# p1an-lin-jung/WavThruVec_pytorch

Measured on AMD Instinct MI355X. Metric: audio samples/sec (16 kHz) Vec2Wav generator, B=32×256-frame 768-d latents, 1/2/4/8 GPU, higher is better.
Workload: dtype f32; 1 GPU; BASELINE configs[1]: B=32/GPU x T=256 frames, 768-d latents, upsample (5,4,4,2,2) x320, ResBlock2, train-mode CondBN, f32; global_batch=32, frames=256, parallelism=single GPU

## Files before the change

include/vec2wav_hip.h:

```cpp
#ifndef VEC2WAV_HIP_H
#define VEC2WAV_HIP_H

#include <stdint.h>

#ifdef __cplusplus
extern "C" {
#endif

#define V2W_ABI_VERSION 34

#define V2W_E_ARG      (-1)
#define V2W_E_SHAPE    (-2)
#define V2W_E_ALGO     (-3)

#define V2W_ALGO_AUTO   0
#define V2W_ALGO_DIRECT 1
#define V2W_ALGO_MFMA   2
#define V2W_ALGO_BF16   4
#define V2W_ALGO_SPLIT  3

int         v2w_abi_version(void);
const char* v2w_build_arch(void);

typedef struct { uint64_t magic; char* buf; int32_t cap; int32_t len; } v2w_name_sink;
#define V2W_NAME_SINK_MAGIC 0x5632574e414d4531ull
#define V2W_NAME_SINK_STREAM(sink) ((void*)((uintptr_t)(sink) | (uintptr_t)1))

int v2w_wn_fold_conv (const float* v, const float* g, float* wf, float* scratch,
                      int c_out, int c_in, int k, void* stream);
int v2w_wn_fold_convt(const float* v, const float* g, float* wf, float* scratch,
                      int c_in, int c_out, int k, void* stream);

int v2w_wf_transpose_flip(const float* wf, float* out, int k, int c_in, int c_out, void* stream);
int v2w_wf_gather_transpose(const float* wf, float* out, int k, int c_in, int c_out, int t_start, int t_step, int n, void* stream);

int v2w_pack_mfma(const float* wf, float* wp, int k, int c_in, int c_out, int u, void* stream);
int v2w_pack_mfma_dgrad(const float* wf, float* wp, int k, int c_in, int c_out, void* stream);
int v2w_pack_mfma_batch(const float* wf, float* wp, int k, int c_in, int c_out, int u, int n, void* stream);

typedef struct {
    const float* v; const float* g; float* wp; float* scale;
    int32_t c_in, c_out, k, u, transposed;
    int32_t mf, ck;
    int32_t _pad;
    float* wf;
    float* wpd;
} v2w_fold_desc;
int v2w_fold_plan(v2w_fold_desc* descs, int n, int32_t* starts);
int v2w_fold_pack_batch(const v2w_fold_desc* descs_dev, const int32_t* starts_dev, int n,
                        int nblk_scale, int nblk_pack, int lds_bytes, void* stream);

typedef struct {
    const float* in;   const float* in_a;  const float* in_s;
    const float* wf;
    const float* wp;
    const float* bias;
    const float* res;  const float* res_a; const float* res_s;
    const float* add0; const float* add1;
    const float* mask_src; const float* mask_a; const float* mask_s;
    float*       out;
    int32_t B, C_in, C_out, L, k, dil;
    float   slope;
    int32_t accumulate;
    float   out_div;
    int32_t algo;
    float   mask_slope;
    int32_t in_stride, in_phase;
    int32_t pad_left;
    const void*  wps;
    const float* winv;
    int32_t in_ct, out_ct;
    float   out_slope;
    int32_t io_bf16;
    float*  rowsum_part;
    float*  splitk_ws;
    int64_t splitk_ws_bytes;
} v2w_conv1d_args;
int v2w_conv1d_fwd(const v2w_conv1d_args* a, void* stream);
long long v2w_conv1d_splitk_ws_bytes(const v2w_conv1d_args* a, int n);
int v2w_conv1d_fwd_multi(const v2w_conv1d_args* a, int n, void* stream);

int v2w_split_supported(int c_in, int c_out, int u);
int v2w_split_packable(int c_in, int c_out);
int v2w_pack_split(const float* wf, void* wps, float* sc, int k, int c_in, int c_out, void* stream);
int v2w_pack_bf16(const float* wf, void* wps, float* sc, int k, int c_in, int c_out, void* stream);
typedef struct {
    const float* v; const float* g;
    void* wps; float* sc;
    float* rowscale;
    int32_t c_in, c_out, k;
    int32_t mode;
} v2w_split_desc;
int v2w_split_pack_batch(const v2w_split_desc* descs_dev, const int32_t* starts_dev, int n, int nblk_rows, int nblk_pack,
                         int k_max, int all_bf16, void* stream);

typedef struct {
    const float* in; const float* in_a; const float* in_s;
    const float* wp1; const float* bias1; const float* wp2; const float* bias2;
    const float* add0; const float* add1;
    float* out;
    int32_t B, C, L, k, dil1, dil2;
    int32_t res_mode;
    float slope, out_div;
} v2w_pair_args;
int v2w_resblock_pair_fwd(const v2w_pair_args* a, int n, void* stream);

typedef struct {
    const float* in; const float* in_a; const float* in_s;
    const float* wp1[4]; const float* bias1[4]; const float* wp2[4]; const float* bias2[4];
    int32_t k[4], dil1[4], dil2[4];
    float* out;
    int32_t nk, B, C, L;
    float slope, out_div;
    const float* post_w; const float* post_b; float* post_out;
    int32_t post_k;
    float post_slope;
    const float* bwd_mask1[4]; float* bwd_mid[4];
    const float* bwd_mask2; const float* bwd_mask2_a; const float* bwd_mask2_s;
    float bwd_slope;
    float* bwd_rowsum[4];
} v2w_stage_args;
int v2w_resblock2_stage_fwd(const v2w_stage_args* a, void* stream);
int v2w_resblock2_stage_bwd_rows(const v2w_stage_args* a);
int v2w_resblock2_stage_small_fwd(const v2w_stage_args* a, void* stream);

typedef struct {
    const float* in; const float* in_a; const float* in_s;
    const void*  wps1[4]; const float* sc1[4]; const float* bias1[4];
    const void*  wps2[4]; const float* sc2[4]; const float* bias2[4];
    int32_t k[4], dil1[4], dil2[4];
    float* out;
    int32_t nk, B, C, L;
    float slope, out_div;
    int32_t bf16;
    int32_t io_bf16;
    const float* post_w; const float* post_b; float* post_out;
    int32_t post_k;
    float post_slope;
    const void* up_wps; const float* up_bias; void* up_out; float* up_stats_part;
    int32_t up_k, up_u;
    float up_slope;
    int32_t rb1;
    const void* in_b[4]; void* out_b[4];
    const void* add0; const void* add1;
} v2w_stage_split_args;
int v2w_resblock2_stage_split_fwd(const v2w_stage_split_args* a, void* stream);
int v2w_resblock2_stage_split_config(const v2w_stage_split_args* a);
int v2w_resblock2_stage_up_tiles(const v2w_stage_split_args* a);

typedef struct {
    const void* in[3];
    const float* in_a; const float* in_s;
    const void* wps[3]; const float* bias[3];
    void* out[3];
    int32_t k[3], dil[3];
    int32_t nbr, mode, B, C, L;
    float slope, out_div;
    int32_t _pad;
} v2w_branch_convs_args;
int v2w_branch_convs_bf16_fwd(const v2w_branch_convs_args* a, void* stream);

typedef struct {
    const float* in; const float* wf; const float* wp; const float* bias; float* out;
    float* stats_part;
    int32_t B, C_in, C_out, L, k, u;
    float   slope;
    int32_t algo;
    int32_t io_bf16;
    int32_t _pad;
    float*  splitk_ws;
    int64_t splitk_ws_bytes;
} v2w_convt1d_args;
int v2w_convt1d_fwd(const v2w_convt1d_args* a, void* stream);
long long v2w_convt1d_splitk_ws_bytes(const v2w_convt1d_args* a);

int       v2w_pack_bf16_convt(const float* wf, void* wps, int k, int c_in, int c_out, int u, void* stream);
long long v2w_pack_bf16_convt_bytes(int k, int c_in, int c_out, int u);
int       v2w_convt1d_bf16_fwd(const v2w_convt1d_args* a, void* stream);
int       v2w_convt1d_bf16_tiles(const v2w_convt1d_args* a);

int v2w_conv1d_tile_config(const v2w_conv1d_args* a, int32_t* cfg);
int v2w_convt1d_tile_config(const v2w_convt1d_args* a, int32_t* cfg);
int v2w_conv1d_bf16_config(const v2w_conv1d_args* a, int n, int32_t* cfg);
int v2w_convt1d_bf16_config(const v2w_convt1d_args* a, int32_t* cfg);

#define V2W_MAX_STAGES 8
typedef struct {
    const float* spk; const float* noise;
    const float* fc_w[V2W_MAX_STAGES]; const float* fc_b[V2W_MAX_STAGES];
    const float* sn_w[V2W_MAX_STAGES]; const float* sn_b[V2W_MAX_STAGES];
    float* sn_u[V2W_MAX_STAGES]; float* sn_v[V2W_MAX_STAGES];
    float* gb[V2W_MAX_STAGES];
    int32_t C[V2W_MAX_STAGES];
    float* z_ws; float* sigma_ws;
    int32_t n_stages, B, spk_dim, noise_dim, training;
} v2w_cond_args;
int v2w_cond_gamma_beta(const v2w_cond_args* a, void* stream);
int v2w_cond_sigma(const v2w_cond_args* a, void* stream);
typedef struct {
// ... 83 lines not shown
```

wavthruvec_pytorch_amd/_hip.py:

```python
from __future__ import annotations

import ctypes as C
import os
import threading

from . import build as _build

ABI_VERSION = 34
V2W_MAX_STAGES = 8
V2W_BN_SPLITS = 64
ALGO_AUTO, ALGO_DIRECT, ALGO_MFMA, ALGO_SPLIT, ALGO_BF16 = 0, 1, 2, 3, 4

_fp = C.c_void_p


class Conv1dArgs(C.Structure):
    _fields_ = [('in_', _fp), ('in_a', _fp), ('in_s', _fp), ('wf', _fp), ('wp', _fp), ('bias', _fp),
                ('res', _fp), ('res_a', _fp), ('res_s', _fp), ('add0', _fp), ('add1', _fp),
                ('mask_src', _fp), ('mask_a', _fp), ('mask_s', _fp), ('out', _fp),
                ('B', C.c_int32), ('C_in', C.c_int32), ('C_out', C.c_int32), ('L', C.c_int32),
                ('k', C.c_int32), ('dil', C.c_int32), ('slope', C.c_float), ('accumulate', C.c_int32),
                ('out_div', C.c_float), ('algo', C.c_int32), ('mask_slope', C.c_float),
                ('in_stride', C.c_int32), ('in_phase', C.c_int32), ('pad_left', C.c_int32),
                ('wps', _fp), ('winv', _fp), ('in_ct', C.c_int32), ('out_ct', C.c_int32), ('out_slope', C.c_float),
                ('io_bf16', C.c_int32), ('rowsum_part', _fp), ('splitk_ws', _fp), ('splitk_ws_bytes', C.c_int64)]


class ConvT1dArgs(C.Structure):
    _fields_ = [('in_', _fp), ('wf', _fp), ('wp', _fp), ('bias', _fp), ('out', _fp), ('stats_part', _fp),
                ('B', C.c_int32), ('C_in', C.c_int32), ('C_out', C.c_int32), ('L', C.c_int32),
                ('k', C.c_int32), ('u', C.c_int32), ('slope', C.c_float), ('algo', C.c_int32), ('io_bf16', C.c_int32), ('_pad', C.c_int32),
                ('splitk_ws', _fp), ('splitk_ws_bytes', C.c_int64)]


class PairArgs(C.Structure):
    _fields_ = [('in_', _fp), ('in_a', _fp), ('in_s', _fp), ('wp1', _fp), ('bias1', _fp), ('wp2', _fp), ('bias2', _fp),
                ('add0', _fp), ('add1', _fp), ('out', _fp),
                ('B', C.c_int32), ('C', C.c_int32), ('L', C.c_int32), ('k', C.c_int32), ('dil1', C.c_int32), ('dil2', C.c_int32),
                ('res_mode', C.c_int32), ('slope', C.c_float), ('out_div', C.c_float)]


class StageArgs(C.Structure):
    _fields_ = [('in_', _fp), ('in_a', _fp), ('in_s', _fp),
                ('wp1', _fp * 4), ('bias1', _fp * 4), ('wp2', _fp * 4), ('bias2', _fp * 4),
                ('k', C.c_int32 * 4), ('dil1', C.c_int32 * 4), ('dil2', C.c_int32 * 4),
                ('out', _fp), ('nk', C.c_int32), ('B', C.c_int32), ('C', C.c_int32), ('L', C.c_int32),
                ('slope', C.c_float), ('out_div', C.c_float),
                ('post_w', _fp), ('post_b', _fp), ('post_out', _fp), ('post_k', C.c_int32), ('post_slope', C.c_float),
                ('bwd_mask1', _fp * 4), ('bwd_mid', _fp * 4), ('bwd_mask2', _fp), ('bwd_mask2_a', _fp), ('bwd_mask2_s', _fp),
                ('bwd_slope', C.c_float), ('bwd_rowsum', _fp * 4)]


class FoldDesc(C.Structure):
    _fields_ = [('v', _fp), ('g', _fp), ('wp', _fp), ('scale', _fp),
                ('c_in', C.c_int32), ('c_out', C.c_int32), ('k', C.c_int32), ('u', C.c_int32), ('transposed', C.c_int32),
                ('mf', C.c_int32), ('ck', C.c_int32), ('_pad', C.c_int32), ('wf', _fp), ('wpd', _fp)]


_P4 = _fp * 4
_I4 = C.c_int32 * 4


class StageSplitArgs(C.Structure):
    _fields_ = [('in_', _fp), ('in_a', _fp), ('in_s', _fp),
                ('wps1', _P4), ('sc1', _P4), ('bias1', _P4), ('wps2', _P4), ('sc2', _P4), ('bias2', _P4),
                ('k', _I4), ('dil1', _I4), ('dil2', _I4), ('out', _fp),
                ('nk', C.c_int32), ('B', C.c_int32), ('C', C.c_int32), ('L', C.c_int32),
                ('slope', C.c_float), ('out_div', C.c_float), ('bf16', C.c_int32), ('io_bf16', C.c_int32),
                ('post_w', _fp), ('post_b', _fp), ('post_out', _fp), ('post_k', C.c_int32), ('post_slope', C.c_float),
                ('up_wps', _fp), ('up_bias', _fp), ('up_out', _fp), ('up_stats_part', _fp),
                ('up_k', C.c_int32), ('up_u', C.c_int32), ('up_slope', C.c_float), ('rb1', C.c_int32),
                ('in_b', _P4), ('out_b', _P4), ('add0', _fp), ('add1', _fp)]


class BranchConvsArgs(C.Structure):
    _fields_ = [('in_', _fp * 3), ('in_a', _fp), ('in_s', _fp), ('wps', _fp * 3), ('bias', _fp * 3), ('out', _fp * 3),
                ('k', C.c_int32 * 3), ('dil', C.c_int32 * 3),
                ('nbr', C.c_int32), ('mode', C.c_int32), ('B', C.c_int32), ('C', C.c_int32), ('L', C.c_int32),
                ('slope', C.c_float), ('out_div', C.c_float), ('_pad', C.c_int32)]


class SplitDesc(C.Structure):
    _fields_ = [('v', _fp), ('g', _fp), ('wps', _fp), ('sc', _fp), ('rowscale', _fp),
                ('c_in', C.c_int32), ('c_out', C.c_int32), ('k', C.c_int32), ('mode', C.c_int32)]


_PA = _fp * V2W_MAX_STAGES


class CondArgs(C.Structure):
    _fields_ = [('spk', _fp), ('noise', _fp),
                ('fc_w', _PA), ('fc_b', _PA), ('sn_w', _PA), ('sn_b', _PA), ('sn_u', _PA), ('sn_v', _PA),
                ('gb', _PA), ('C', C.c_int32 * V2W_MAX_STAGES), ('z_ws', _fp), ('sigma_ws', _fp),
                ('n_stages', C.c_int32), ('B', C.c_int32), ('spk_dim', C.c_int32), ('noise_dim', C.c_int32),
                ('training', C.c_int32)]


class CondEvalArgs(C.Structure):
    _fields_ = [('c', CondArgs), ('running_mean', _PA), ('running_var', _PA), ('a_out', _PA), ('s_out', _PA),
                ('eps', C.c_float * V2W_MAX_STAGES)]


SIGNATURES = {
    'v2w_abi_version': (C.c_int, []),
    'v2w_build_arch': (C.c_char_p, []),
    'v2w_wn_fold_conv': (C.c_int, [_fp, _fp, _fp, _fp, C.c_int, C.c_int, C.c_int, _fp]),
    'v2w_wn_fold_convt': (C.c_int, [_fp, _fp, _fp, _fp, C.c_int, C.c_int, C.c_int, _fp]),
    'v2w_wf_transpose_flip': (C.c_int, [_fp, _fp, C.c_int, C.c_int, C.c_int, _fp]),
    'v2w_wf_gather_transpose': (C.c_int, [_fp, _fp, C.c_int, C.c_int, C.c_int, C.c_int, C.c_int, C.c_int, _fp]),
    'v2w_pack_mfma': (C.c_int, [_fp, _fp, C.c_int, C.c_int, C.c_int, C.c_int, _fp]),
    'v2w_pack_mfma_batch': (C.c_int, [_fp, _fp, C.c_int, C.c_int, C.c_int, C.c_int, C.c_int, _fp]),
    'v2w_pack_mfma_dgrad': (C.c_int, [_fp, _fp, C.c_int, C.c_int, C.c_int, _fp]),
    'v2w_split_supported': (C.c_int, [C.c_int, C.c_int, C.c_int]),
    'v2w_pack_split': (C.c_int, [_fp, _fp, _fp, C.c_int, C.c_int, C.c_int, _fp]),
    'v2w_mel_phases': (C.c_int, [_fp, _fp, C.c_int, C.c_int, C.c_int, C.c_int, C.c_int, _fp]),
    'v2w_mel_finish': (C.c_int, [_fp, _fp, _fp, C.c_int, C.c_int, C.c_int, C.c_int, C.c_int, C.c_int, _fp]),
    'v2w_mel_finish_bwd': (C.c_int, [_fp, _fp, _fp, _fp, _fp, C.c_int, C.c_int, C.c_int, C.c_int, C.c_int, C.c_int, _fp]),
    'v2w_phase_split': (C.c_int, [_fp, _fp, C.c_int, C.c_int, C.c_int, C.c_int, C.c_int, C.c_int, C.c_int, C.c_int, _fp]),
    'v2w_unfold1': (C.c_int, [_fp, _fp, C.c_int, C.c_int, C.c_int, C.c_int, C.c_int, C.c_int, C.c_int, C.c_int, C.c_int, _fp]),
    'v2w_unfold_taps': (C.c_int, [_fp, _fp] + [C.c_int] * 9 + [_fp]),
    'v2w_wgrad_slice': (C.c_int, [_fp, _fp, _fp, _fp] + [C.c_int] * 9 + [_fp]),
    'v2w_wgrad_group_slabs': (C.c_int, [C.c_int] * 5),
    'v2w_wgrad_groups': (C.c_int, [_fp, _fp, _fp, _fp] + [C.c_int] * 8 + [_fp]),
    'v2w_disc_dz': (C.c_int, [_fp, _fp, _fp, _fp, _fp, C.c_longlong, C.c_int, C.c_int, C.c_float, _fp]),
    'v2w_rowsum_reduce': (C.c_int, [_fp, _fp, C.c_int, C.c_int, _fp]),
    'v2w_disc_dz_merge': (C.c_int, [_fp, _fp, _fp, _fp, _fp] + [C.c_int] * 8 + [C.c_float, _fp]),
    'v2w_phase_merge': (C.c_int, [_fp, _fp] + [C.c_int] * 8 + [_fp]),
    'v2w_fold1': (C.c_int, [_fp, _fp] + [C.c_int] * 9 + [_fp]),
    'v2w_avgpool4_bwd': (C.c_int, [_fp, _fp, C.c_int, C.c_int, _fp]),
    'v2w_cout1_wgrad': (C.c_int, [_fp, _fp, _fp] + [C.c_int] * 6 + [_fp]),
    'v2w_zero_tail': (C.c_int, [_fp, C.c_longlong, C.c_int, C.c_int, _fp]),
    'v2w_avgpool4': (C.c_int, [_fp, _fp, C.c_int, C.c_int, _fp]),
    'v2w_mel_phases_bwd': (C.c_int, [_fp, _fp, C.c_int, C.c_int, C.c_int, C.c_int, C.c_int, _fp]),
    'v2w_split_packable': (C.c_int, [C.c_int, C.c_int]),
    'v2w_resblock2_stage_split_fwd': (C.c_int, [C.POINTER(StageSplitArgs), _fp]),
    'v2w_resblock2_stage_split_config': (C.c_int, [C.POINTER(StageSplitArgs)]),
    'v2w_resblock2_stage_up_tiles': (C.c_int, [C.POINTER(StageSplitArgs)]),
    'v2w_pack_bf16': (C.c_int, [_fp, _fp, _fp, C.c_int, C.c_int, C.c_int, _fp]),
    'v2w_split_pack_batch': (C.c_int, [_fp, _fp, C.c_int, C.c_int, C.c_int, C.c_int, C.c_int, _fp]),
    'v2w_fold_plan': (C.c_int, [C.POINTER(FoldDesc), C.c_int, C.POINTER(C.c_int32)]),
    'v2w_fold_pack_batch': (C.c_int, [_fp, _fp, C.c_int, C.c_int, C.c_int, C.c_int, _fp]),
    'v2w_conv1d_fwd': (C.c_int, [C.POINTER(Conv1dArgs), _fp]),
    'v2w_conv1d_fwd_multi': (C.c_int, [C.POINTER(Conv1dArgs), C.c_int, _fp]),
    'v2w_conv1d_splitk_ws_bytes': (C.c_longlong, [C.POINTER(Conv1dArgs), C.c_int]),
    'v2w_convt1d_splitk_ws_bytes': (C.c_longlong, [C.POINTER(ConvT1dArgs)]),
    'v2w_resblock_pair_fwd': (C.c_int, [C.POINTER(PairArgs), C.c_int, _fp]),
    'v2w_resblock2_stage_bwd_rows': (C.c_int, [C.POINTER(StageArgs)]),
    'v2w_resblock2_stage_fwd': (C.c_int, [C.POINTER(StageArgs), _fp]),
    'v2w_resblock2_stage_small_fwd': (C.c_int, [C.POINTER(StageArgs), _fp]),
    'v2w_branch_convs_bf16_fwd': (C.c_int, [C.POINTER(BranchConvsArgs), _fp]),
    'v2w_convt1d_fwd': (C.c_int, [C.POINTER(ConvT1dArgs), _fp]),
    'v2w_pack_bf16_convt': (C.c_int, [_fp, _fp, C.c_int, C.c_int, C.c_int, C.c_int, _fp]),
    'v2w_pack_bf16_convt_bytes': (C.c_longlong, [C.c_int, C.c_int, C.c_int, C.c_int]),
    'v2w_convt1d_bf16_fwd': (C.c_int, [C.POINTER(ConvT1dArgs), _fp]),
    'v2w_convt1d_bf16_tiles': (C.c_int, [C.POINTER(ConvT1dArgs)]),
    'v2w_conv1d_tile_config': (C.c_int, [C.POINTER(Conv1dArgs), C.POINTER(C.c_int32)]),
    'v2w_convt1d_tile_config': (C.c_int, [C.POINTER(ConvT1dArgs), C.POINTER(C.c_int32)]),
    'v2w_conv1d_bf16_config': (C.c_int, [C.POINTER(Conv1dArgs), C.c_int, C.POINTER(C.c_int32)]),
    'v2w_convt1d_bf16_config': (C.c_int, [C.POINTER(ConvT1dArgs), C.POINTER(C.c_int32)]),
    'v2w_cond_gamma_beta': (C.c_int, [C.POINTER(CondArgs), _fp]),
    'v2w_cond_sigma': (C.c_int, [C.POINTER(CondArgs), _fp]),
    'v2w_cond_affine_eval': (C.c_int, [C.POINTER(CondEvalArgs), _fp]),
    'v2w_bn_stats': (C.c_int, [_fp, _fp, _fp, C.c_int, C.c_int, C.c_int, _fp]),
    'v2w_bn_reduce_partials': (C.c_int, [_fp, C.c_int, C.c_int, C.c_double, _fp, _fp]),
    'v2w_bn_finalize': (C.c_int, [_fp, _fp, _fp, _fp, _fp, _fp, _fp, C.c_int, C.c_int, C.c_int,
                                  C.c_float, C.c_float, _fp]),
    'v2w_bn_reduce_finalize': (C.c_int, [_fp, C.c_int, C.c_double, _fp, _fp, _fp, _fp, _fp, _fp, _fp, C.c_int, C.c_int, C.c_float, C.c_float, _fp]),
    'v2w_bn_reduce_slices': (C.c_int, [_fp, C.c_int, C.c_int, _fp, C.c_int, _fp]),
    'v2w_bn_finalize_slices': (C.c_int, [_fp, C.c_int, C.c_double, _fp, _fp, _fp, _fp, _fp, _fp, C.c_int, C.c_int, C.c_float, C.c_float, _fp]),
    'v2w_affine_apply': (C.c_int, [_fp, _fp, _fp, _fp, C.c_int, C.c_int, C.c_int, _fp]),
    'v2w_wgrad_slabs': (C.c_int, [C.c_int, C.c_int, C.c_int, C.c_int]),
    'v2w_wgrad': (C.c_int, [_fp, _fp, _fp, _fp, _fp, _fp, C.c_int, C.c_int, C.c_int, C.c_int, C.c_int, C.c_int, C.c_int,
                            C.c_float, _fp]),
    'v2w_wgrad_bf16_slabs': (C.c_int, [C.c_int] * 5),
    'v2w_wgrad_bf16': (C.c_int, [_fp] * 6 + [C.c_int] * 6 + [C.c_float, C.c_int, _fp]),
    'v2w_cbn_bwd_sums': (C.c_int, [_fp] * 9 + [C.c_int, C.c_int, C.c_int, C.c_int, C.c_float, _fp]),
    'v2w_cbn_bwd_apply': (C.c_int, [_fp] * 9 + [C.c_int, C.c_int, C.c_int, C.c_int, C.c_float, _fp]),
    'v2w_tail_bwd': (C.c_int, [_fp] * 8 + [C.c_int, C.c_int, C.c_int, C.c_int, C.c_float, _fp]),
    'v2w_wn_bwd': (C.c_int, [_fp] * 5 + [C.c_int, C.c_int, C.c_int, C.c_int, _fp]),
    'v2w_cond_bwd': (C.c_int, [_fp] * 13 + [C.c_int, C.c_int, C.c_int, C.c_int, _fp]),
    'v2w_conv_post_tanh_bf16in': (C.c_int, [_fp, _fp, _fp, _fp, C.c_int, C.c_int, C.c_int, C.c_int, C.c_float, _fp]),
    'v2w_conv_post_tanh': (C.c_int, [_fp, _fp, _fp, _fp, C.c_int, C.c_int, C.c_int, C.c_int, C.c_float, _fp]),
}

LAUNCHERS = frozenset(n for n, (_r, a) in SIGNATURES.items() if a and a[-1] is _fp)

_lib = None
_tls = threading.local()


class HipLibraryError(RuntimeError):

    def __init__(self, msg, code=None):
        super().__init__(msg)
        self.code = code


E_ARG, E_SHAPE, E_ALGO = -1, -2, -3


def lib_path() -> str:
    return os.environ.get('V2W_LIB') or _build.LIB_PATH


def load():
    global _lib
    rec = getattr(_tls, 'recorder', None)
    if rec is not None:
        return rec
    if _lib is not None:
        return _lib
    import torch
    path = lib_path()
    if not os.path.exists(path):
        raise HipLibraryError(
            f'{path} not found: build it with `python -m wavthruvec_pytorch_amd.build` '
            '(or __graft_entry__.build()); there is no CPU/PyTorch fallback for the Vec2Wav hot path')
    lib = C.CDLL(path)
    for name, (res, args) in SIGNATURES.items():
        try:
            fn = getattr(lib, name)
        except AttributeError as e:
            raise HipLibraryError(f'{path} does not export {name}') from e
        fn.restype = res
        fn.argtypes = args
    if lib.v2w_abi_version() != ABI_VERSION:
        raise HipLibraryError(f'ABI version mismatch: library {lib.v2w_abi_version()}, binding {ABI_VERSION}')
    _lib = lib
    return lib


def set_recorder(rec):
    prev = getattr(_tls, 'recorder', None)
    _tls.recorder = rec
    return prev


class NameSink(C.Structure):
    _fields_ = [('magic', C.c_uint64), ('buf', C.c_void_p), ('cap', C.c_int32), ('len', C.c_int32)]


NAME_SINK_MAGIC = 0x5632574e414d4531


def kernel_name_short(full: str) -> str:
    s = full.strip()
    if s.startswith('void '):
        s = s[5:]
    s = s.replace('(anonymous namespace)::', '')
    depth = 0
    for i, ch in enumerate(s):
        if ch == '<':
            depth += 1
        elif ch == '>':
            depth -= 1
        elif ch == '(' and depth == 0:
            return s[:i]
    return s


def kernel_names(fn, *args, short=True):
    buf = C.create_string_buffer(8192)
    sink = NameSink(NAME_SINK_MAGIC, C.addressof(buf), len(buf), 0)
    rc = fn(*args, C.c_void_p(C.addressof(sink) | 1))
    names = [n for n in buf.value.decode().split('\n') if n]
# ... 34 lines not shown
```

wavthruvec_pytorch_amd/build.py:

```python
from __future__ import annotations

import contextlib
import fcntl
import hashlib
import os
import shutil
import subprocess
from concurrent.futures import ThreadPoolExecutor

PKG_DIR = os.path.dirname(os.path.abspath(__file__))
CSRC = os.path.join(PKG_DIR, 'csrc')
OBJ_DIR = os.path.join(CSRC, '_obj')
LIB_PATH = os.path.join(PKG_DIR, 'libvec2wav_hip.so')
SOURCES = ['v2w_api.hip', 'v2w_conv_mfma.hip', 'v2w_conv_split.hip', 'v2w_conv_bf16.hip', 'v2w_conv_bf16_res.hip', 'v2w_convt_bf16_res.hip', 'v2w_stage_split.hip', 'v2w_stage_bf16.hip', 'v2w_stage_bf16_wide.hip', 'v2w_stage_bf16_n16.hip', 'v2w_stage_bf16_n16s.hip', 'v2w_stage_bf16_n32s.hip', 'v2w_resblock_fused.hip', 'v2w_stage_small.hip',
           'v2w_wgrad.hip', 'v2w_wgrad_bf16.hip', 'v2w_backward.hip', 'v2w_direct.hip', 'v2w_conv_post_bf16.hip', 'v2w_cbn.hip', 'v2w_fold.hip', 'v2w_mel.hip', 'v2w_disc.hip']
HEADERS = ['v2w_common.h', 'v2w_tile.h', os.path.join('..', '..', 'include', 'vec2wav_hip.h')]
FLAGS = ['--offload-arch=gfx950', '-O3', '-std=c++17', '-fPIC']


def find_hipcc() -> str:
    for cand in (os.environ.get('HIPCC'), shutil.which('hipcc'), '/opt/rocm/bin/hipcc'):
        if cand and os.path.exists(cand):
            return cand
    raise RuntimeError('hipcc not found (set HIPCC or install ROCm)')


def _obj(src: str) -> str:
    return os.path.join(OBJ_DIR, src + '.o')


def _stale_sources():
    hdr_t = max(os.path.getmtime(os.path.join(CSRC, h)) for h in HEADERS)
    out = []
    for s in SOURCES:
        o = _obj(s)
        if not os.path.exists(o) or os.path.getmtime(o) < max(hdr_t, os.path.getmtime(os.path.join(CSRC, s))):
            out.append(s)
    return out


def needs_build() -> bool:
    if not os.path.exists(LIB_PATH):
        return True
    t = os.path.getmtime(LIB_PATH)
    deps = [os.path.join(CSRC, s) for s in SOURCES + HEADERS]
    return any(os.path.getmtime(d) > t for d in deps)


def sources_hash() -> str:
    hsh = hashlib.sha256()
    for f in sorted(SOURCES) + sorted(HEADERS):
        with open(os.path.join(CSRC, f), 'rb') as fh:
            hsh.update(os.path.basename(f).encode() + b'\0' + fh.read())
    return hsh.hexdigest()[:16]


@contextlib.contextmanager
def _build_lock():
    os.makedirs(OBJ_DIR, exist_ok=True)
    with open(os.path.join(OBJ_DIR, '.lock'), 'w') as lk:
        fcntl.flock(lk, fcntl.LOCK_EX)
        try:
            yield
        finally:
            fcntl.flock(lk, fcntl.LOCK_UN)


def build(force: bool = False, verbose: bool = False, jobs: int | None = None) -> str:
    if not force and not needs_build():
        return LIB_PATH
    hipcc = find_hipcc()
    with _build_lock():
        if not force and not needs_build():
            return LIB_PATH
        todo = list(SOURCES) if force else _stale_sources()

        def run(cmd, what):
            if verbose:
                print(' '.join(cmd), flush=True)
            r = subprocess.run(cmd, capture_output=True, text=True)
            if r.returncode != 0:
                raise RuntimeError(f'{what}:\n' + r.stdout + r.stderr)

        def compile_one(s):
            tmp = _obj(s) + f'.tmp{os.getpid()}'
            try:
                run([hipcc] + FLAGS + ['-c', '-o', tmp, os.path.join(CSRC, s)], f'hipcc failed on {s}')
                os.replace(tmp, _obj(s))
            finally:
                if os.path.exists(tmp):
                    os.remove(tmp)

        jobs = jobs or max(1, min(len(todo) or 1, (os.cpu_count() or 2)))
        with ThreadPoolExecutor(max_workers=jobs) as ex:
            list(ex.map(compile_one, todo))
        tmp = LIB_PATH + f'.tmp{os.getpid()}'
        try:
            run([hipcc, '--offload-arch=gfx950', '-fPIC', '-shared', '-o', tmp] + [_obj(s) for s in SOURCES], 'hipcc link failed')
            os.replace(tmp, LIB_PATH)
        finally:
            if os.path.exists(tmp):
                os.remove(tmp)
    return LIB_PATH


if __name__ == '__main__':
    import sys
    print(build(force='--force' in sys.argv, verbose=True))
```

wavthruvec_pytorch_amd/csrc/v2w_api.hip:

```cpp
#include "v2w_common.h"

int v2w_conv1d_mfma(const v2w_conv1d_args* a, int n, hipStream_t stream, int* cfg_out, long long* ws_query = nullptr);
int v2w_convt1d_mfma(const v2w_convt1d_args* a, hipStream_t stream, int* cfg_out, long long* ws_query = nullptr);
int v2w_conv1d_split(const v2w_conv1d_args* a, int n, hipStream_t stream, bool bf16);
int v2w_conv1d_direct(const v2w_conv1d_args* a, hipStream_t stream);
int v2w_convt1d_direct(const v2w_convt1d_args* a, hipStream_t stream);

extern "C" int v2w_abi_version(void) { return V2W_ABI_VERSION; }
extern "C" const char* v2w_build_arch(void) { return "gfx950"; }

static int check_conv1d(const v2w_conv1d_args* a) {
    if (!a || !a->in || !a->out) return V2W_E_ARG;
    if ((a->algo == V2W_ALGO_SPLIT || a->algo == V2W_ALGO_BF16) ? (!a->wps || !a->winv) : (!a->wf && !a->wp)) return V2W_E_ARG;
    if (a->B <= 0 || a->C_in <= 0 || a->C_out <= 0 || a->L <= 0 || a->k <= 0 || a->dil <= 0) return V2W_E_ARG;
    if ((a->k & 1) == 0 && a->pad_left < 0) return V2W_E_SHAPE;
    if (a->pad_left > a->dil * (a->k - 1) || a->in_stride < 0 || a->in_phase < 0 || (a->in_stride > 0 && a->in_phase >= a->in_stride))
        return V2W_E_ARG;
    if ((a->in_a == nullptr) != (a->in_s == nullptr)) return V2W_E_ARG;
    if ((a->res_a == nullptr) != (a->res_s == nullptr)) return V2W_E_ARG;
    if (a->res_a && !a->res) return V2W_E_ARG;
    if (a->add1 && !a->add0) return V2W_E_ARG;
    if (a->add0 && a->accumulate) return V2W_E_ARG;
    if ((a->mask_a == nullptr) != (a->mask_s == nullptr)) return V2W_E_ARG;
    if (a->mask_a && !a->mask_src) return V2W_E_ARG;
    if (a->in_ct < 0 || a->out_ct < 0 || (a->in_ct > 0 && a->in_ct < a->C_in) || (a->out_ct > 0 && a->out_ct < a->C_out)) return V2W_E_ARG;
    if (((a->in_ct > 0 && a->in_ct != a->C_in) && a->in_a) || ((a->out_ct > 0 && a->out_ct != a->C_out) && (a->res_a || a->mask_a)))
        return V2W_E_ARG;
    if (a->out_slope < 0.f) return V2W_E_ARG;
    if (a->rowsum_part && (a->algo != V2W_ALGO_MFMA || !a->mask_src)) return V2W_E_ARG;
    if (a->io_bf16 != 0 && (a->algo != V2W_ALGO_BF16 || a->io_bf16 < 0 || a->io_bf16 > 3)) return V2W_E_ARG;
    const bool ext_ct = (a->in_ct > 0 && a->in_ct != a->C_in) || (a->out_ct > 0 && a->out_ct != a->C_out);
    const bool ext_slope = a->out_slope != 0.f && a->out_slope != 1.f;
    if ((ext_ct || ext_slope) && a->algo == V2W_ALGO_BF16) return V2W_E_SHAPE;
    return 0;
}

extern "C" int v2w_conv1d_fwd(const v2w_conv1d_args* a, void* stream) {
    if (const int rc = check_conv1d(a)) return rc;
    hipStream_t st = (hipStream_t)stream;
    switch (a->algo) {
        case V2W_ALGO_DIRECT: return a->wf ? v2w_conv1d_direct(a, st) : V2W_E_ARG;
        case V2W_ALGO_MFMA: return v2w_conv1d_mfma(a, 1, st, nullptr);
        case V2W_ALGO_SPLIT: return v2w_conv1d_split(a, 1, st, false);
        case V2W_ALGO_BF16: return v2w_conv1d_split(a, 1, st, true);
        case V2W_ALGO_AUTO: {
            const int rc = v2w_conv1d_mfma(a, 1, st, nullptr);
            return rc == V2W_E_SHAPE ? (a->wf ? v2w_conv1d_direct(a, st) : V2W_E_ARG) : rc;
        }
        default: return V2W_E_ALGO;
    }
}

extern "C" int v2w_convt1d_fwd(const v2w_convt1d_args* a, void* stream) {
    if (!a || !a->in || (!a->wf && !a->wp) || !a->out || a->io_bf16 != 0) return V2W_E_ARG;
    if (a->B <= 0 || a->C_in <= 0 || a->C_out <= 0 || a->L <= 0 || a->k <= 0 || a->u <= 0) return V2W_E_ARG;
    if (a->k < a->u || ((a->k - a->u) & 1)) return V2W_E_SHAPE;
    hipStream_t st = (hipStream_t)stream;
    switch (a->algo) {
        case V2W_ALGO_DIRECT: return (a->wf && !a->stats_part) ? v2w_convt1d_direct(a, st) : V2W_E_ARG;
        case V2W_ALGO_MFMA: return v2w_convt1d_mfma(a, st, nullptr);
        case V2W_ALGO_AUTO: {
            const int rc = v2w_convt1d_mfma(a, st, nullptr);
            return rc == V2W_E_SHAPE ? ((a->wf && !a->stats_part) ? v2w_convt1d_direct(a, st) : V2W_E_ARG) : rc;
        }
        default: return V2W_E_ALGO;
    }
}

extern "C" int v2w_conv1d_tile_config(const v2w_conv1d_args* a, int32_t* cfg) {
    if (!a || !cfg) return V2W_E_ARG;
    return v2w_conv1d_mfma(a, 1, nullptr, cfg);
}
extern "C" int v2w_convt1d_tile_config(const v2w_convt1d_args* a, int32_t* cfg) {
    if (!a || !cfg) return V2W_E_ARG;
    return v2w_convt1d_mfma(a, nullptr, cfg);
}

extern "C" long long v2w_conv1d_splitk_ws_bytes(const v2w_conv1d_args* a, int n) {
    if (!a || n < 1 || n > 4 || (a->algo != V2W_ALGO_AUTO && a->algo != V2W_ALGO_MFMA)) return 0;
    long long bytes = 0;
    return v2w_conv1d_mfma(a, n, nullptr, nullptr, &bytes) == 0 ? bytes : 0;
}
extern "C" long long v2w_convt1d_splitk_ws_bytes(const v2w_convt1d_args* a) {
    if (!a || a->u <= 0 || a->k < a->u || (a->algo != V2W_ALGO_AUTO && a->algo != V2W_ALGO_MFMA)) return 0;
    long long bytes = 0;
    return v2w_convt1d_mfma(a, nullptr, nullptr, &bytes) == 0 ? bytes : 0;
}

extern "C" int v2w_conv1d_fwd_multi(const v2w_conv1d_args* a, int n, void* stream) {
    if (!a || n < 1 || n > 4) return V2W_E_ARG;
    for (int i = 0; i < n; ++i) {
        if (const int rc = check_conv1d(a + i)) return rc;
        if (a[i].algo == V2W_ALGO_DIRECT) return V2W_E_SHAPE;
        if (a[i].algo != a[0].algo && (a[i].algo >= V2W_ALGO_SPLIT || a[0].algo >= V2W_ALGO_SPLIT)) return V2W_E_ARG;
    }
    if (a[0].algo == V2W_ALGO_SPLIT || a[0].algo == V2W_ALGO_BF16)
        return v2w_conv1d_split(a, n, (hipStream_t)stream, a[0].algo == V2W_ALGO_BF16);
    return v2w_conv1d_mfma(a, n, (hipStream_t)stream, nullptr);
}
```

wavthruvec_pytorch_amd/csrc/v2w_conv_mfma.hip:

```cpp
#include <type_traits>
#include "v2w_tile.h"

#ifdef V2W_TIMELINE
V2W_TL_SETTER(v2w_timeline_set_tile)
#endif

namespace {

template <int MF, int CK> struct TileGeom {
    static constexpr int RS = CK == 32 ? 36 : (MF == 32 ? 20 : 24);
    static constexpr int PAIR_DC = MF == 32 ? 2 : 4;
    __host__ __device__ static constexpr int slot(int c) {
        return MF == 32 ? ((c & ~7) + 4 * (c & 1) + ((c & 7) >> 1)) : (4 * (c & 3) + (c >> 2));
    }
    __host__ __device__ static constexpr int pair_c0(int P) {
        return MF == 32 ? (8 * (P >> 2) + 4 * (P & 1) + ((P >> 1) & 1)) : (8 * (P & 1) + (P >> 1));
    }
};

template <int MF, int U, int MI, int NI, int WM, int WN, int CK, int NPF, int RING, int EPI, bool VEC>
__global__ void __launch_bounds__(64 * WM * WN, (U == 1 && MI * NI >= 4) ? 3 : 1)
conv_tile_kernel(const MultiArgs m) {
    typedef Frag<MF> F;
    typedef typename F::acc_t acc_t;
    constexpr int NTHREADS = 64 * WM * WN;
    constexpr int MT = MF * MI * WM;
    constexpr int NT = MF * NI * WN;
    constexpr int KSTEP = F::KSTEP;
    constexpr int CKG = 4 * KSTEP;
    constexpr int GPC = CK / CKG;
    constexpr int RS = TileGeom<MF, CK>::RS;
    static_assert(CK % CKG == 0, "chunk must hold whole A fragments");
    static_assert(RING == 2 || (RING == 4 && GPC == 4), "the 4-deep ring walks exactly one tap per revolution");

    extern __shared__ __attribute__((aligned(16))) float smem[];

    int pq = 0;
#pragma unroll
    for (int i = 1; i < V2W_MAX_MULTI; ++i) pq += (int)blockIdx.x >= m.start[i] ? 1 : 0;
    const TileArgs& p = m.p[pq];
    const int mtiles = p.Cout / MT;
    int id = blockIdx.x - m.start[pq];
    int slice = 0;
    if (p.ksplit > 1) {
        const int per = ((p.ntiles + 7) >> 3) * 8 * mtiles;
        slice = id / per;
        id -= slice * per;
    }
    const int grp = id / (8 * mtiles), rem = id % (8 * mtiles);
    const int mt = rem >> 3;
    const int tile = grp * 8 + (rem & 7);
    if (tile >= p.ntiles) return;
    const int b = tile / p.ntl;
    const int n0 = (tile % p.ntl) * NT;
    const int m0 = mt * MT;

    const int tid = threadIdx.x;
    const int lane = tid & 63;
    const int wave = __builtin_amdgcn_readfirstlane(tid >> 6);
    const int lr = lane & (MF - 1);
    const int hk = lane / MF;
    const int wm0 = (wave / WN) * (MF * MI);
    const int wn0 = (wave % WN) * (MF * NI);
    const int L = p.L, K = p.K;
    const float slope = p.slope;
    const int nch = p.Cin / CK;
    const int nchs = p.ksplit > 1 ? nch / p.ksplit : nch;
    const int ch0 = slice * nchs, ch1 = ch0 + nchs;
    float* const outp = p.out + (size_t)slice * p.B * p.CoutT * L * U;
    const int pos0 = n0 - p.hla;
    const int bufsz = p.xrows * RS;
    float* const etab = smem + p.atab_off;
    float* const atab = etab + 5 * MT;

    V2W_STAMP(0);
    acc_t acc[U][MI][NI];
#pragma unroll
    for (int r = 0; r < U; ++r)
#pragma unroll
        for (int i = 0; i < MI; ++i)
#pragma unroll
            for (int j = 0; j < NI; ++j)
#pragma unroll
                for (int e = 0; e < F::NREG; ++e) acc[r][i][j][e] = 0.f;

    const int nq = p.xrows >> 2;
    const int nq8 = (nq + 7) >> 3;
    const unsigned magic = (unsigned)(((1ull << 32) + nq8 - 1) / nq8);
    f32x4 pf[NPF][2];
    const f32x4 zero4 = {0.f, 0.f, 0.f, 0.f};
    auto item = [&](int s, int& c0, int& row, bool& in_img, bool& in_seq) {
        int t = tid;
        asm volatile("" : "+v"(t));
        const int idx = t + s * NTHREADS;
        const int g = idx >> 4;
        const int pg = (int)__umulhi((unsigned)g, magic);
        const int quad = (g - pg * nq8) * 8 + (idx & 7);
        const int P = 2 * pg + ((idx >> 3) & 1);
        row = quad * 4;
        in_img = quad < nq && P < CK / 2;
        c0 = TileGeom<MF, CK>::pair_c0(in_img ? P : 0);
        const int pos = pos0 + row;
        in_seq = in_img && pos >= 0 && pos < L;
    };
    auto prefetch = [&](int ci0) {
        const float* src = p.in + (size_t)(b * p.CinT + ci0) * L + pos0;
#pragma unroll
        for (int s = 0; s < NPF; ++s) {
            int c0, row; bool in_img, in_seq;
            item(s, c0, row, in_img, in_seq);
            pf[s][0] = zero4; pf[s][1] = zero4;
            if (in_seq) {
                pf[s][0] = *reinterpret_cast<const f32x4*>(src + (size_t)c0 * L + row);
                pf[s][1] = *reinterpret_cast<const f32x4*>(src + (size_t)(c0 + TileGeom<MF, CK>::PAIR_DC) * L + row);
            }
        }
    };
    auto commit = [&](int ci0, float* Xs) {
#pragma unroll
        for (int s = 0; s < NPF; ++s) {
            int c0, row; bool in_img, in_seq;
            item(s, c0, row, in_img, in_seq);
            if (!in_img) continue;
            float a0 = 1.f, s0 = 0.f, a1 = 1.f, s1 = 0.f;
            if (p.in_a) {
                a0 = atab[ci0 + c0]; s0 = atab[p.Cin + ci0 + c0];
                a1 = atab[ci0 + c0 + TileGeom<MF, CK>::PAIR_DC]; s1 = atab[p.Cin + ci0 + c0 + TileGeom<MF, CK>::PAIR_DC];
            }
            float* dst = Xs + row * RS + TileGeom<MF, CK>::slot(c0);
#pragma unroll
            for (int e = 0; e < 4; ++e) {
                f32x2 v = {0.f, 0.f};
                if (in_seq) { v[0] = v2w_lrelu(fmaf(a0, pf[s][0][e], s0), slope); v[1] = v2w_lrelu(fmaf(a1, pf[s][1][e], s1), slope); }
                *reinterpret_cast<f32x2*>(dst + e * RS) = v;
            }
        }
    };
    auto stage_scalar = [&](int ci0, float* Xs) {
        for (int c = wave; c < CK; c += WM * WN) {
            const int ch = b * p.CinT + ci0 + c;
            const float* src = p.in + (size_t)ch * L * p.in_stride + p.in_phase;
            const float av = p.in_a ? p.in_a[ch] : 1.f;
            const float sv = p.in_s ? p.in_s[ch] : 0.f;
            float* dst = Xs + TileGeom<MF, CK>::slot(c);
            for (int j = lane; j < p.xrows; j += 64) {
                const int l = pos0 + j;
                float v = 0.f;
                if (l >= 0 && l < L) v = v2w_lrelu(fmaf(av, src[(size_t)l * p.in_stride], sv), slope);
                dst[j * RS] = v;
            }
        }
    };

    const int nfrag = nch * K * GPC;
// ... 475 lines not shown
            floats += n * s2;
        }
        if (m.p[0].ws_query) {
            *m.p[0].ws_query = ok ? (long long)(floats * sizeof(float)) : 0;
            return 0;
        }
        if (ok && m.p[0].splitk_ws && (long long)(floats * sizeof(float)) <= m.p[0].splitk_ws_bytes) {
            float* ws = m.p[0].splitk_ws;
            {
                S = s2;
                red_vec = vec;
                size_t off = 0;
                long long f4 = 0;
                grid = 0;
                for (int i = 0; i < nprob; ++i) {
                    TileArgs& p = m.p[i];
                    const size_t n = (size_t)p.B * p.Cout * p.L * U;
                    red.e[i] = SplitEpi{ws + off, p.out, p.bias, p.res, p.res_a, p.res_s, p.add0, p.add1, p.accumulate, p.out_div, p.Cout, p.L * U, n};
                    red.start[i] = f4;
                    f4 += vec ? (long long)(n / 4) : (long long)p.B * p.Cout * p.L * U;
                    p.out = ws + off; p.bias = nullptr; p.res = p.res_a = p.res_s = nullptr; p.add0 = p.add1 = nullptr;
                    p.accumulate = 0; p.out_div = 0.f; p.ksplit = S;
                    p.evec = U == 1 && p.L % 4 == 0;
                    off += n * S;
                    m.start[i] = grid;
                    grid += ((p.ntiles + 7) / 8) * 8 * (p.Cout / MT) * S;
                }
                m.start[nprob] = grid;
                red.start[nprob] = f4;
                red.n = nprob; red.S = S;
            }
        }
    }
    if (m.p[0].ws_query) { *m.p[0].ws_query = 0; return 0; }
    bool vec = true;
    for (int i = 0; i < nprob; ++i) vec = vec && m.p[i].vec4;
    auto kern = vec ? (epi == 1 ? conv_tile_kernel<MF, U, MI, NI, WM, WN, CK, NPF, RING, 1, true>
                       : (epi == 2 ? conv_tile_kernel<MF, U, MI, NI, WM, WN, CK, NPF, RING, 2, true> : conv_tile_kernel<MF, U, MI, NI, WM, WN, CK, NPF, RING, 0, true>))
                    : (epi == 1 ? conv_tile_kernel<MF, U, MI, NI, WM, WN, CK, NPF, RING, 1, false>
                       : (epi == 2 ? conv_tile_kernel<MF, U, MI, NI, WM, WN, CK, NPF, RING, 2, false> : conv_tile_kernel<MF, U, MI, NI, WM, WN, CK, NPF, RING, 0, false>));
    if (lds > 64 * 1024) {
        if (lds > 160 * 1024) return V2W_E_SHAPE;
        hipError_t e = v2w_max_lds(reinterpret_cast<const void*>(kern), (int)lds, stream);
        if (e != hipSuccess) return (int)e;
    }
    V2W_LAUNCH(kern, dim3(grid), dim3(NTHREADS), lds, stream, m);
    if (S > 1) {
        const int rc = v2w_launch_status();
        if (rc != 0) return rc;
        long long blocks = (red.start[nprob] + 255) / 256;
        if (blocks > 2048) blocks = 2048;
        if (red_vec) V2W_LAUNCH(splitk_reduce_kernel<true>, dim3((int)blocks), dim3(256), 0, stream, red);
        else V2W_LAUNCH(splitk_reduce_kernel<false>, dim3((int)blocks), dim3(256), 0, stream, red);
    }
    return v2w_launch_status();
}

template <int U>
int launch_convt_u(TileArgs p, hipStream_t stream) {
    if (p.Cout % 64 == 0) return launch_tile<32, U, 1, 1, 2, 2, 16>(&p, 1, stream);
    if (p.Cout == 32) return launch_tile<32, U, 1, 1, 1, 4, 16>(&p, 1, stream);
    if (p.Cout == 16) return launch_tile<16, U, 1, 2, 1, 4, 16>(&p, 1, stream);
    return V2W_E_SHAPE;
}

__global__ void __launch_bounds__(256)
pack_mfma_kernel(const float* wf, float* wp, int K, int Cin, int Cout, int MF, int CK, int U, int tflip = 0) {
    const int KSTEP = MF == 32 ? 2 : 4, CKG = 4 * KSTEP, GPC = CK / CKG, nch = Cin / CK;
    const int pad = (K - U) / 2;
    const size_t total = (size_t)K * Cin * Cout;
    wf += (size_t)blockIdx.y * total; wp += (size_t)blockIdx.y * total;
    for (size_t o = (size_t)blockIdx.x * 256 + threadIdx.x; o < total; o += (size_t)gridDim.x * 256) {
        const int j = o & 3;
        const int lane = (o >> 2) & 63;
        size_t rest = o >> 8;
        const int gg = rest % GPC; rest /= GPC;
        const int ts = rest % K; rest /= K;
        const int ch = rest % nch;
        const int mb = rest / nch;
        int t = ts;
        if (U > 1) {
            int left = ts;
            for (int r = 0; r < U; ++r) {
                const int t0 = (r + pad) % U, nt = (K - t0 + U - 1) / U;
                if (left < nt) { t = t0 + left * U; break; }
                left -= nt;
            }
        }
        const int c = ch * CK + gg * CKG + j * KSTEP + lane / MF;
        const int co = mb * MF + lane % MF;
        wp[o] = tflip ? wf[((size_t)(K - 1 - t) * Cout + co) * Cin + c] : wf[((size_t)t * Cin + c) * Cout + co];
    }
}


__device__ __forceinline__ int find_layer(const int32_t* __restrict__ starts, int n, int blk) {
    int lo = 0, hi = n;
    while (hi - lo > 1) { const int mid = (lo + hi) >> 1; if (starts[mid] <= blk) lo = mid; else hi = mid; }
    return lo;
}

__global__ void __launch_bounds__(256)
fold_scale_batch_kernel(const v2w_fold_desc* __restrict__ descs, const int32_t* __restrict__ starts, int n) {
    __shared__ double red[16];
    const int li = find_layer(starts, n, blockIdx.x);
    const v2w_fold_desc d = descs[li];
    const int row = blockIdx.x - starts[li];
    const int inner = (d.transposed ? d.c_out : d.c_in) * d.k;
    const float* src = d.v + (size_t)row * inner;
    double acc = 0.0;
    if (d.g)
        for (int i = threadIdx.x; i < inner; i += 256) { const double x = (double)src[i]; acc += x * x; }
    const double n2 = v2w_block_sum(acc, red);
    if (threadIdx.x == 0) d.scale[row] = d.g ? (float)((double)d.g[row] / sqrt(n2)) : 1.f;
}

__global__ void __launch_bounds__(256)
fold_pack_batch_kernel(const v2w_fold_desc* __restrict__ descs, const int32_t* __restrict__ starts, int n) {
    extern __shared__ float tile[];
    const int li = find_layer(starts, n, blockIdx.x);
    const v2w_fold_desc d = descs[li];
    const int blk = blockIdx.x - starts[li];
    const int MF = d.mf, CK = d.ck, K = d.k, U = d.u;
    const int KSTEP = MF == 32 ? 2 : 4, CKG = 4 * KSTEP, GPC = CK / CKG, nch = d.c_in / CK;
    const int mb = blk / nch, ch = blk % nch;
    const int nrow = d.transposed ? CK : MF;
    const int rlen = (d.transposed ? MF : CK) * K;
    const int rstride = rlen + 1;
    for (int idx = threadIdx.x; idx < nrow * rlen; idx += 256) {
        const int r = idx / rlen, x = idx - r * rlen;
        const float* src = d.transposed ? d.v + ((size_t)(ch * CK + r) * d.c_out + mb * MF) * K
                                        : d.v + ((size_t)(mb * MF + r) * d.c_in + ch * CK) * K;
        const float sc = d.scale[d.transposed ? ch * CK + r : mb * MF + r];
        tile[r * rstride + x] = src[x] * sc;
    }
    __syncthreads();
    const int pad = (K - U) / 2;
    float* dst = d.wp + (size_t)(mb * nch + ch) * K * GPC * 256;
    for (int o = threadIdx.x; o < K * GPC * 256; o += 256) {
        const int j = o & 3, lane = (o >> 2) & 63;
        const int rest = o >> 8;
        const int gg = rest % GPC, ts = rest / GPC;
        int t = ts;
        if (U > 1) {
            int left = ts;
            for (int r = 0; r < U; ++r) {
                const int t0 = (r + pad) % U, nt = (K - t0 + U - 1) / U;
                if (left < nt) { t = t0 + left * U; break; }
                left -= nt;
            }
        }
        const int c = gg * CKG + j * KSTEP + lane / MF, co = lane % MF;
        dst[o] = d.transposed ? tile[c * rstride + co * K + t] : tile[co * rstride + c * K + t];
    }
    if (d.wf) {
        for (int idx = threadIdx.x; idx < K * CK * MF; idx += 256) {
            const int col = idx % MF, c = (idx / MF) % CK, t = idx / (MF * CK);
            d.wf[((size_t)t * d.c_in + ch * CK + c) * d.c_out + mb * MF + col] =
                d.transposed ? tile[c * rstride + col * K + t] : tile[col * rstride + c * K + t];
        }
    }
    if (d.wpd) {
        const int nchd = d.c_out / CK;
        float* dd = d.wpd + (size_t)(ch * nchd + mb) * K * GPC * 256;
        for (int o = threadIdx.x; o < K * GPC * 256; o += 256) {
            const int j = o & 3, lane = (o >> 2) & 63;
            const int rest = o >> 8;
            const int gg = rest % GPC, ts = rest / GPC;
            const int kc = gg * CKG + j * KSTEP + lane / MF, row = lane % MF;
            dd[o] = tile[kc * rstride + row * K + (K - 1 - ts)];
        }
    }
}

}

struct LayerCfg { int mf, ck; };
static LayerCfg v2w_layer_cfg(int c_in, int c_out, int u) {
    LayerCfg c{0, 0};
    if (c_in % 16 != 0) return c;
    if (u == 1) {
        if (c_out % 32 == 0 && c_in % 32 == 0) c = {32, 32};
        else if (c_out % 32 == 0) c = {32, 16};
        else if (c_out == 16) c = {16, 16};
    } else if (u == 2 || u == 4 || u == 5 || u == 8) {
        if (c_out % 64 == 0 || c_out == 32) c = {32, 16};
        else if (c_out == 16) c = {16, 16};
    }
    return c;
}

extern "C" int v2w_pack_mfma(const float* wf, float* wp, int k, int c_in, int c_out, int u, void* stream) {
    if (!wf || !wp || k <= 0 || c_in <= 0 || c_out <= 0 || u <= 0) return V2W_E_ARG;
    const LayerCfg cfg = v2w_layer_cfg(c_in, c_out, u);
    if (!cfg.mf) return V2W_E_SHAPE;
    const size_t total = (size_t)k * c_in * c_out;
    int grid = (int)((total + 255) / 256); if (grid > 4096) grid = 4096;
    V2W_LAUNCH(pack_mfma_kernel, dim3(grid), dim3(256), 0, (hipStream_t)stream, wf, wp, k, c_in, c_out, cfg.mf, cfg.ck, u);
    return v2w_launch_status();
}

extern "C" int v2w_pack_mfma_dgrad(const float* wf, float* wp, int k, int c_in, int c_out, void* stream) {
    if (!wf || !wp || k <= 0 || c_in <= 0 || c_out <= 0) return V2W_E_ARG;
    const LayerCfg cfg = v2w_layer_cfg(c_in, c_out, 1);
    if (!cfg.mf) return V2W_E_SHAPE;
    const size_t total = (size_t)k * c_in * c_out;
    int grid = (int)((total + 255) / 256); if (grid > 4096) grid = 4096;
    V2W_LAUNCH(pack_mfma_kernel, dim3(grid), dim3(256), 0, (hipStream_t)stream, wf, wp, k, c_in, c_out, cfg.mf, cfg.ck, 1, 1);
    return v2w_launch_status();
}

extern "C" int v2w_pack_mfma_batch(const float* wf, float* wp, int k, int c_in, int c_out, int u, int n, void* stream) {
    if (n <= 0 || n > 65535) return V2W_E_ARG;
    if (!wf || !wp || k <= 0 || c_in <= 0 || c_out <= 0 || u <= 0) return V2W_E_ARG;
    const LayerCfg cfg = v2w_layer_cfg(c_in, c_out, u);
    if (!cfg.mf) return V2W_E_SHAPE;
    const size_t total = (size_t)k * c_in * c_out;
    int grid = (int)((total + 255) / 256); if (grid > 4096) grid = 4096;
    V2W_LAUNCH(pack_mfma_kernel, dim3(grid, n), dim3(256), 0, (hipStream_t)stream, wf, wp, k, c_in, c_out, cfg.mf, cfg.ck, u);
    return v2w_launch_status();
}

int v2w_conv1d_mfma(const v2w_conv1d_args* a, int n, hipStream_t stream, int* cfg_out, long long* ws_query) {
    if (n < 1 || n > V2W_MAX_MULTI) return V2W_E_ARG;
    const LayerCfg cfg = v2w_layer_cfg(a->C_in, a->C_out, 1);
    if (!cfg.mf) return V2W_E_SHAPE;
    TileArgs ps[V2W_MAX_MULTI];
    long tiles128 = 0;
    for (int i = 0; i < n; ++i) {
        const v2w_conv1d_args* q = a + i;
        if (q->B != a->B || q->C_in != a->C_in || q->C_out != a->C_out || q->L != a->L) return V2W_E_SHAPE;
        if (!q->wp && !cfg_out && !ws_query) return V2W_E_SHAPE;
        TileArgs p{};
        p.cfg_out = cfg_out;
        p.in = q->in; p.in_a = q->in_a; p.in_s = q->in_s; p.wp = q->wp; p.bias = q->bias;
        p.res = q->res; p.res_a = q->res_a; p.res_s = q->res_s; p.out = q->out;
        p.add0 = q->add0; p.add1 = q->add1;
        p.mask_src = q->mask_src; p.mask_a = q->mask_a; p.mask_s = q->mask_s; p.mask_slope = q->mask_slope;
        p.stats_part = q->rowsum_part;
        p.B = q->B; p.Cin = q->C_in; p.Cout = q->C_out; p.L = q->L; p.K = q->k; p.dil = q->dil;
        p.CinT = q->in_ct > 0 ? q->in_ct : q->C_in; p.CoutT = q->out_ct > 0 ? q->out_ct : q->C_out;
        p.out_slope = q->out_slope > 0.f ? q->out_slope : 1.f;
        p.pad = 0; p.hl = p.hr = q->dil * (q->k - 1) / 2;
        if (q->pad_left >= 0) { p.hl = q->pad_left; p.hr = q->dil * (q->k - 1) - q->pad_left; if (p.hr < 0) return V2W_E_ARG; }
        p.in_stride = q->in_stride > 0 ? q->in_stride : 1; p.in_phase = q->in_phase;
        p.slope = q->slope; p.accumulate = q->accumulate; p.out_div = q->out_div;
        p.splitk_ws = a->splitk_ws; p.splitk_ws_bytes = a->splitk_ws ? a->splitk_ws_bytes : 0; p.ws_query = ws_query;
        ps[i] = p;
        tiles128 += (long)p.B * ((p.L + 127) / 128) * (p.Cout / 128);
    }
    int halo = 0;
    for (int i = 0; i < n; ++i) { const int h = ((ps[i].hl + 3) & ~3) > ps[i].hr ? ((ps[i].hl + 3) & ~3) : ps[i].hr; if (h > halo) halo = h; }
    if (halo > 32) {
        if (halo > 48 || cfg.mf != 32 || cfg.ck != 32 || a->C_out % 64 != 0) return V2W_E_SHAPE;
        if (a->C_out % 128 == 0 && tiles128 >= 4 * 256) return launch_tile<32, 1, 2, 2, 2, 2, 32, 48>(ps, n, stream);
        return launch_tile<32, 1, 1, 2, 2, 2, 32, 48>(ps, n, stream);
    }
    if (cfg.mf == 32 && cfg.ck == 32 && a->C_out % 64 == 0 && (long)n * a->B * ((a->L + 63) / 64) * (a->C_out / 64) < 512)
        return launch_tile<32, 1, 1, 1, 2, 2, 32>(ps, n, stream);
    if (cfg.mf == 32 && cfg.ck == 32 && a->C_out % 128 == 0) {
        if (tiles128 >= 4 * 256) return launch_tile<32, 1, 2, 2, 2, 2, 32>(ps, n, stream);
        return launch_tile<32, 1, 2, 1, 2, 2, 32>(ps, n, stream);
    }
    if (cfg.mf == 32 && cfg.ck == 32 && a->C_out % 64 == 0) return launch_tile<32, 1, 1, 2, 2, 2, 32>(ps, n, stream);
    if (cfg.mf == 32 && cfg.ck == 16) return launch_tile<32, 1, 1, 2, 1, 4, 16>(ps, n, stream);
    if (cfg.mf == 32) return launch_tile<32, 1, 1, 2, 1, 4, 32>(ps, n, stream);
    if (cfg.mf == 16) return launch_tile<16, 1, 1, 4, 1, 4, 16>(ps, n, stream);
    return V2W_E_SHAPE;
}

int v2w_convt1d_mfma(const v2w_convt1d_args* a, hipStream_t stream, int* cfg_out, long long* ws_query) {
    const LayerCfg cfg = v2w_layer_cfg(a->C_in, a->C_out, a->u);
    if ((!a->wp && !cfg_out && !ws_query) || !cfg.mf) return V2W_E_SHAPE;
    TileArgs p{};
    p.cfg_out = cfg_out;
    p.splitk_ws = a->splitk_ws; p.splitk_ws_bytes = a->splitk_ws ? a->splitk_ws_bytes : 0; p.ws_query = ws_query;
    p.in = a->in; p.wp = a->wp; p.bias = a->bias; p.out = a->out; p.stats_part = a->stats_part;
    p.B = a->B; p.Cin = a->C_in; p.Cout = a->C_out; p.L = a->L; p.K = a->k; p.dil = 1;
    p.CinT = p.Cin; p.CoutT = p.Cout; p.out_slope = 1.f;
    p.pad = (a->k - a->u) / 2;
    p.slope = a->slope; p.accumulate = 0; p.out_div = 0.f;
    int hl = 0, hr = 0;
    for (int r = 0; r < a->u; ++r) {
        const int rp = r + p.pad, t0 = rp % a->u, c = rp / a->u, nt = (a->k - t0 + a->u - 1) / a->u;
        if (c > hr) hr = c;
        if (nt - 1 - c > hl) hl = nt - 1 - c;
    }
    p.hl = hl; p.hr = hr;
    switch (a->u) {
        case 2: return launch_convt_u<2>(p, stream);
        case 4: return launch_convt_u<4>(p, stream);
        case 5: return launch_convt_u<5>(p, stream);
        case 8: return launch_convt_u<8>(p, stream);
        default: return V2W_E_SHAPE;
    }
}

extern "C" int v2w_fold_plan(v2w_fold_desc* descs, int n, int32_t* starts) {
    if (!descs || !starts || n <= 0) return V2W_E_ARG;
    int bs = 0, bp = 0, lds = 0;
    for (int i = 0; i < n; ++i) {
        v2w_fold_desc& d = descs[i];
        if (d.c_in <= 0 || d.c_out <= 0 || d.k <= 0 || d.u <= 0) return V2W_E_ARG;
        const LayerCfg cfg = v2w_layer_cfg(d.c_in, d.c_out, d.transposed ? d.u : 1);
        if (!cfg.mf) return V2W_E_SHAPE;
        d.mf = cfg.mf; d.ck = cfg.ck;
        if (d.wpd && (d.transposed || d.c_in != d.c_out || cfg.mf != cfg.ck)) return V2W_E_ARG;
        starts[i] = bs; starts[n + 1 + i] = bp;
        bs += d.transposed ? d.c_in : d.c_out;
        bp += (d.c_out / cfg.mf) * (d.c_in / cfg.ck);
        const int nrow = d.transposed ? cfg.ck : cfg.mf, rlen = (d.transposed ? cfg.mf : cfg.ck) * d.k;
        const int bytes = nrow * (rlen + 1) * (int)sizeof(float);
        if (bytes > lds) lds = bytes;
    }
    starts[n] = bs; starts[2 * n + 1] = bp;
    if (lds > 160 * 1024) return V2W_E_SHAPE;
    return lds;
}

extern "C" int v2w_fold_pack_batch(const v2w_fold_desc* descs_dev, const int32_t* starts_dev, int n,
                                   int nblk_scale, int nblk_pack, int lds_bytes, void* stream) {
    if (!descs_dev || !starts_dev || n <= 0 || nblk_scale <= 0 || nblk_pack <= 0 || lds_bytes <= 0) return V2W_E_ARG;
    hipStream_t st = (hipStream_t)stream;
    if (lds_bytes > 64 * 1024) {
        hipError_t e = v2w_max_lds(reinterpret_cast<const void*>(fold_pack_batch_kernel), lds_bytes, st);
        if (e != hipSuccess) return (int)e;
    }
    V2W_LAUNCH(fold_scale_batch_kernel, dim3(nblk_scale), dim3(256), 0, st, descs_dev, starts_dev, n);
    V2W_LAUNCH(fold_pack_batch_kernel, dim3(nblk_pack), dim3(256), lds_bytes, st, descs_dev, starts_dev + n + 1, n);
    return v2w_launch_status();
}
```

wavthruvec_pytorch_amd/forward_plan.py:

```python
from __future__ import annotations

import contextlib

import torch

from . import hipops

LRELU_SLOPE = 0.1
_Z_CHANNEL = 128


class DirectStreams:

    def __init__(self, main, side, side2=None):
        self.main, self.side, self.side2 = main, side, side if side2 is None else side2
        self.events = {}
        self.nfork = 1
        self.tag = None

    def stream(self, sid):
        return (self.main, self.side, self.side2)[sid]

    def fork(self, sides=1):
        self.nfork = sides
# ... 36 lines not shown
        self.order = []
        self.needed = set()

    def run(self):
        g = self.g
        keep_ws = None
        if self.save is not None:
            keep_ws, g._ws = g._ws, {}
        try:
            with torch.no_grad():
                self.begin()
                self.weights()
                self.conv_pre()
                for i in range(self.ns):
                    self.stage(i)
                y = self.tail()
            if self.save is not None:
                self.hand_over(y)
        finally:
            if keep_ws is not None:
                g._ws = keep_ws
        return y

    def timed(self, tag, fn, *args, **kw):
        g = self.g
        self.S.tag = tag
        try:
            if g._profile is None or not isinstance(self.S, DirectStreams):
                return fn(*args, **kw)
            e0, e1 = torch.cuda.Event(enable_timing=True), torch.cuda.Event(enable_timing=True)
            pn = g._profile_names
            e0.record()
            if pn is not None:
                from . import _hip, schedule
                prev = _hip.set_recorder(schedule.NameProbe(_hip.load(), pn.setdefault(tag, [])))
                try:
                    r = fn(*args, **kw)
                finally:
                    _hip.set_recorder(prev)
            else:
                r = fn(*args, **kw)
            e1.record()
            g._profile.append((tag, e0, e1))
            return r
        finally:
            self.S.tag = None

    def on_side(self, sid=1):
        return torch.cuda.stream(self.S.stream(sid))

    def mark(self, name, sid=1):
        self.S.mark(name, sid)
        self.marked.add(name)
        self.order.append((name, sid))

    def need(self, *names):
        want = [nm for nm in names if nm in self.marked and nm not in self.needed]
        if not self.g.merge_waits:
            for nm in want:
                self.needed.add(nm)
                self.S.need(nm)
            return
        for sid in sorted({s for n, s in self.order if n in want}):
            seq = [n for n, s in self.order if s == sid]
            last = max(seq.index(n) for n in want if n in seq)
            self.S.need(seq[last])
            self.needed.update(seq[:last + 1])

    def join_side(self):
        if not self.joined:
            self.S.join()
            self.joined = True

    def begin(self):
        g, x = self.g, self.x
        from .models import ResBlock1, ResBlock2
        self.fuse_stage = () if self.save is not None else g.fuse_stage
        self.fuse_pairs = () if self.save is not None else g.fuse_pairs
        self.adt = torch.float32
        rb1_net = all(isinstance(rb, ResBlock1) for rb in g.resblocks)
        if (g.precision == 'bf16' and g.bf16_storage and self.save is None and self.algo == hipops.ALGO_AUTO and self.nk <= 3
                and (all(isinstance(rb, ResBlock2) for rb in g.resblocks) or rb1_net) and x.shape[2] % 4 == 0 and g.h.num_wv_feat % 32 == 0
                and all((up.out_channels >= 64 and up.out_channels % 64 == 0) or up.out_channels in self.fuse_stage for up in g.ups)
                and all(up.in_channels % 32 == 0 and 2 <= up.stride <= 8 for up in g.ups)
                and g._bf16_storage_kernels_exist(self.B, self.T)):
            self.adt = torch.bfloat16
        self.st = self.adt == torch.bfloat16
        cs = g.cond_stream if g.cond_stream is not None else 3072 <= self.B * self.T <= 10240
        self.cond_sid = 2 if (self.st and self.training and cs) else 1
        self.joined = False
        self.S.fork(self.cond_sid)
        self.slab = g._slab(self.dev)
        self.y = None
        self.wps32 = {}
        self.up_done = None

    def buf(self, name, shape, dtype=torch.float32):
        return self.g._buf(name, shape, dtype=dtype, device=self.dev)

    def weights(self):
        g, st, dev = self.g, self.st, self.dev
        B, ns = self.B, self.ns
        self.gbs = [self.buf(f'gb.{i}', (B, 2 * g.cbns[i].num_features)) for i in range(ns)]
        self.z_ws = self.buf('z_ws', (ns * B * _Z_CHANNEL,))
        self.sigma_ws = self.buf('sigma_ws', (ns,))
        self.affs = None
        self.cond_ran = False
        if self.cond_sid == 2:
            self.cond()
        with (self.on_side() if st else contextlib.nullcontext()):
            self.wf, self.wp = g._fold_weights(dev, need_wf=self.save is not None, bf16_only=st)
        self.wps = g._split_weights(dev, all_ups=st, ups_stream=self.S.side, mark=self.mark if st else None,
                                    between=self.cond if st else None)
        self.cond()

    def cond(self):
        if self.cond_ran:
            return
        self.cond_ran = True
        g, dev, ns, B = self.g, self.dev, self.ns, self.B
        with self.on_side(self.cond_sid):
            if not self.training and self.save is None:
                sn_p = [q for c in g.cbns for q in (c.layer.weight_orig, c.layer.weight_u, c.layer.weight_v)]
                skey = (tuple((q.data_ptr(), q._version) for q in sn_p), str(dev))
                if g._fold_key.get('sigma') != skey:
                    hipops.cond_sigma([c.layer.weight_orig.detach() for c in g.cbns], [c.layer.weight_u for c in g.cbns],
                                      [c.layer.weight_v for c in g.cbns], self.sigma_ws, training=False)
                    g._fold_key['sigma'] = skey
                self.affs = [(self.buf(f'bn.a{i}', (B, g.cbns[i].num_features)), self.buf(f'bn.s{i}', (B, g.cbns[i].num_features))) for i in range(ns)]
                hipops.cond_affine_eval(
                    self.spk, self.nz, [f.weight.detach() for f in g.fcs], [f.bias.detach() for f in g.fcs],
                    [c.layer.weight_orig.detach() for c in g.cbns], [c.layer.bias.detach() for c in g.cbns], self.sigma_ws,
                    [c.batch_nrom.running_mean for c in g.cbns], [c.batch_nrom.running_var for c in g.cbns],
                    [c.batch_nrom.eps for c in g.cbns], [q[0] for q in self.affs], [q[1] for q in self.affs])
            else:
                g._fold_key.pop('sigma', None)
                hipops.cond_gamma_beta(
                    self.spk, self.nz, [f.weight.detach() for f in g.fcs], [f.bias.detach() for f in g.fcs],
                    [c.layer.weight_orig.detach() for c in g.cbns], [c.layer.bias.detach() for c in g.cbns],
                    [c.layer.weight_u for c in g.cbns], [c.layer.weight_v for c in g.cbns], self.gbs, self.z_ws, self.sigma_ws, self.training)
        if self.st:
            self.mark('cond', self.cond_sid)

    def ck(self, nm, io=3):
        g = self.g
        if nm in self.wps32:
            return dict(algo=hipops.ALGO_BF16, wps=self.wps32[nm])
        if nm in self.wps and nm in g._split_wide:
            if self.st:
                return dict(algo=hipops.ALGO_BF16, wps=self.wps[nm], io_bf16=io)
            return dict(algo=hipops.ALGO_BF16 if g.precision == 'bf16' else hipops.ALGO_SPLIT, wps=self.wps[nm])
        if self.st:
            raise RuntimeError(f'bf16 storage: layer {nm} has no bf16 kernel (set generator.bf16_storage = False)')
        return dict(algo=self.algo, wp=self.wp[nm])

    def conv_pre(self):
        g = self.g
        self.cur = self.buf('act.pre', (self.B, g.h.upsample_initial_channel, self.T), dtype=self.adt)
        self.timed('conv_pre', hipops.conv1d, self.x, self.wf['conv_pre'], g.conv_pre.bias.detach(), self.cur, k=7, dil=1,
                   slope=1.0, splitk_ws=self.slab, **self.ck('conv_pre', io=2))
        self.L = self.T

    def stage(self, i):
        up = self.g.ups[i]
        self.C, self.Lo = up.out_channels, self.L * up.stride
        self.xr = self.buf(f'act.up{i}', (self.B, self.C, self.Lo), dtype=self.adt)
        nt_stats, part = self.upsample(i)
        self.aff = self.statistics(i, nt_stats, part)
        self.need('rest', f'ups.{i + 1}' if i + 1 < self.ns else 'post')
        self.xs = self.buf(f'act.rb{i}', (self.B, self.C, self.Lo), dtype=self.adt)
        self.residual(i)
        self.cur, self.L = self.xs, self.Lo

    def upsample(self, i):
        g, st, up, C = self.g, self.st, self.g.ups[i], self.C
        B, L, dev = self.B, self.L, self.dev
        if st:
            if self.up_done is None:
                self.need(f'ups.{i}')
        elif f'ups.{i}' in self.wps:
            self.join_side()
        part, nt_stats = None, 0
        if self.training:
            if self.up_done is not None:
                nt_stats = self.up_done
            elif f'ups.{i}' in self.wps:
                nt_stats = hipops.convt_bf16_stats_tiles(self.cur, self.xr, up.kernel_size, up.stride, io_bf16=3 if st else 0)
            elif self.algo != hipops.ALGO_DIRECT and self.wp[f'ups.{i}'] is not None:
                nt_stats = hipops.convt_stats_tiles(B, up.in_channels, C, L, up.kernel_size, up.stride)
            if nt_stats:
                part = self.buf(f'bn.part{i}', (nt_stats * C * 2,))
        if self.up_done is not None:
            pass
        elif f'ups.{i}' in self.wps and (nt_stats or not self.training):
            self.timed(f'ups.{i}', hipops.convt1d_bf16, self.cur, self.wps[f'ups.{i}'], up.bias.detach(), self.xr, k=up.kernel_size,
                       u=up.stride, slope=LRELU_SLOPE, stats_part=part, io_bf16=3 if st else 0)
        elif st:
            raise RuntimeError(f'bf16 storage: ups.{i} has no bf16 kernel (set generator.bf16_storage = False)')
        else:
            self.timed(f'ups.{i}', hipops.convt1d, self.cur, self.wf[f'ups.{i}'], up.bias.detach(), self.xr, k=up.kernel_size,
                       u=up.stride, slope=LRELU_SLOPE, algo=self.algo, wp=self.wp[f'ups.{i}'], stats_part=part, splitk_ws=self.slab)
        self.up_done = None
        return nt_stats, part

    def statistics(self, i, nt_stats, part):
        g, C, B, Lo = self.g, self.C, self.B, self.Lo
        bn = g.cbns[i].batch_nrom
        sliced = self.training and nt_stats >= 4096 and g.stat_sync is None and self.save is None
        stats = None
        fused = g.fuse_bn_finalize and self.training and not sliced and nt_stats and g.stat_sync is None and self.affs is None
        if self.training and not sliced:
            stats = self.buf(f'bn.stats{i}', (2 * C + 1,), dtype=torch.float64)
            if fused:
                pass
            elif nt_stats:
                hipops.bn_reduce_partials(part, nt_stats, C, B * Lo, stats)
            else:
                hipops.bn_stats(self.xr, stats, self.buf('bn.partial', (2 * max(C, 256) * 64,), dtype=torch.float64))
            if g.stat_sync is not None:
                sync = g.stat_sync
                self.timed(f'stat_sync.{i}', self.S.py, lambda: sync(stats))
        a_t, s_t = self.buf(f'bn.a{i}', (B, C)), self.buf(f'bn.s{i}', (B, C))
        self.need('cond')
        if not self.st:
            self.join_side()
        if sliced:
            sl = self.buf(f'bn.slices{i}', (hipops.BN_SLICES * 2 * C,), dtype=torch.float64)
            hipops.bn_reduce_finalize_slices(part, nt_stats, B * Lo, sl, self.gbs[i], bn.running_mean, bn.running_var, bn.num_batches_tracked,
                                             a_t, s_t, momentum=bn.momentum, eps=bn.eps)
        elif fused:
            hipops.bn_reduce_finalize(part, nt_stats, B * Lo, stats, self.gbs[i], bn.running_mean, bn.running_var, bn.num_batches_tracked,
                                      a_t, s_t, momentum=bn.momentum, eps=bn.eps)
        elif self.affs is None:
            hipops.bn_finalize(stats, self.gbs[i], bn.running_mean, bn.running_var, bn.num_batches_tracked, a_t, s_t,
                               training=self.training, momentum=bn.momentum, eps=bn.eps)
        return a_t, s_t

    def residual(self, i):
        from .models import ResBlock2
        g, nk = self.g, self.nk
        self.rbs = [g.resblocks[i * nk + j] for j in range(nk)]
        self.names = [f'resblocks.{i * nk + j}' for j in range(nk)]
        self.wps32 = {}
        if (self.save is not None and g.precision == 'bf16' and not self.st and self.C == 32 and self.Lo % 4 == 0 and self.algo == hipops.ALGO_AUTO
                and all(isinstance(rb, ResBlock2) and rb.kernel_size >= 3 and rb.kernel_size % 2 == 1 for rb in self.rbs)):
            for nm in self.names:
                for c in (0, 1):
                    self.wps32[f'{nm}.convs.{c}'] = hipops.pack_split(self.wf[f'{nm}.convs.{c}'], bf16=True)
        if not (self.algo != hipops.ALGO_DIRECT and nk <= 3):
            return self.residual_serial(i)
        B, C, Lo = self.B, self.C, self.Lo
        self.t1s = [self.buf(f'act.t1_{i}_{j}', (B, C, Lo), dtype=self.adt) for j in range(nk)]
        self.outs = [self.buf(f'act.o_{i}_{j}', (B, C, Lo), dtype=self.adt) for j in range(nk - 1)] + [self.xs]
        self.heavy_first = sorted(range(nk), key=lambda j: -self.rbs[j].kernel_size)
        if not isinstance(self.rbs[0], ResBlock2):
            return self.residual1(i)
        self.all_wps = all(f'{nm}.convs.{c}' in self.wps for nm in self.names for c in (0, 1))
        self.all_wp = all(self.wp.get(f'{nm}.convs.{c}') is not None for nm in self.names for c in (0, 1))
        for cand in (self.rb2_stage_with_upsampler, self.rb2_narrow_stage_split, self.rb2_wide_stage_bf16, self.rb2_stage_f32,
                     self.rb2_stage_small, self.rb2_pairs, self.rb2_branch_convs_bf16, self.rb2_layers):
            if cand(i):
                return
            if self.st and cand is self.rb2_wide_stage_bf16 and C in (16, 32):
                raise RuntimeError('bf16 storage: the fused narrow-stage kernel did not take this shape (set generator.bf16_storage = False)')

    def launch(self, tag_sfx, probs):
        probs = [probs[j] for j in self.heavy_first if j in probs]
        tag = '+'.join(f'{self.names[j]}.{tag_sfx}' for j, _ in probs)
        self.timed(tag, hipops.conv1d_multi, [pr for _, pr in probs], splitk_ws=self.slab)

    def final_kw(self, j):
        if j < self.nk - 1:
            return {}
        return dict(add=self.outs[:self.nk - 1], out_div=float(self.nk))

    def stage_tag(self, sfx=''):
        return 'stage:' + '+'.join(f'{nm}.0&1' for nm in self.names) + sfx

    def rb2_stage_with_upsampler(self, i):
        g, C, B, Lo, rbs = self.g, self.C, self.B, self.Lo, self.rbs
        if not (self.st and g.fuse_up and i + 1 < self.ns and C >= 32 and (C >= 64 and g.fuse_wide_stage or C in self.fuse_stage)
                and f'ups.{i + 1}' in self.wps and self.all_wps):
            return False
        nup = g.ups[i + 1]
        if not (nup.kernel_size == 2 * nup.stride and nup.stride in (2, 4) and nup.out_channels * 2 == C):
            return False
        ntn = hipops.resblock2_stage_up_tiles(B, C, Lo, [rb.kernel_size for rb in rbs], [rb.convs[0].dilation for rb in rbs],
                                              [rb.convs[1].dilation for rb in rbs], slope=LRELU_SLOPE,
                                              up_k=nup.kernel_size, up_u=nup.stride, up_slope=LRELU_SLOPE)
        if not ntn:
            return False
        xr_n = self.buf(f'act.up{i + 1}', (B, nup.out_channels, Lo * nup.stride), dtype=self.adt)
        part_n = self.buf(f'bn.part{i + 1}', (ntn * nup.out_channels * 2,)) if self.training else None
        ok = self.timed(self.stage_tag(f'+ups.{i + 1}'), hipops.resblock2_stage_split, self.xr, self.aff, _branches(rbs, self.names, self.wps), None,
                        slope=LRELU_SLOPE, out_div=float(self.nk), bf16=True, io_bf16=3,
                        up=(self.wps[f'ups.{i + 1}'], nup.bias.detach(), xr_n, part_n, nup.kernel_size, nup.stride, LRELU_SLOPE))
        if ok:
            self.up_done = ntn
        return ok

    def rb2_narrow_stage_split(self, i):
        g, C, B, Lo, rbs = self.g, self.C, self.B, self.Lo, self.rbs
        if not (C in (16, 32) and C in self.fuse_stage and self.all_wps):
            return False
        branches = _branches(rbs, self.names, self.wps)
        std_set = [(rb.kernel_size, rb.convs[0].dilation, rb.convs[1].dilation) for rb in rbs] == [(3, 1, 3), (7, 1, 3), (11, 1, 3)]
# ... 183 lines not shown
```

wavthruvec_pytorch_amd/hipops.py:

```python
from __future__ import annotations

import ctypes as C
from typing import Optional, Sequence

import torch

from . import _hip

ALGO_AUTO, ALGO_DIRECT, ALGO_MFMA, ALGO_SPLIT, ALGO_BF16 = (_hip.ALGO_AUTO, _hip.ALGO_DIRECT, _hip.ALGO_MFMA, _hip.ALGO_SPLIT,
                                                             _hip.ALGO_BF16)


def _chk(t: Optional[torch.Tensor], name: str, dtype=torch.float32):
    if t is None:
        return
    if not t.is_cuda:
        raise RuntimeError(f'{name} must live on a GPU: the Vec2Wav HIP path has no CPU fallback')
    if t.dtype != dtype:
        raise TypeError(f'{name} must be {dtype}, got {t.dtype}')
    if not t.is_contiguous():
        raise RuntimeError(f'{name} must be contiguous')


def _stream(t: torch.Tensor) -> int:
    return torch.cuda.current_stream(t.device).cuda_stream


def fold_conv_weight(v, g, out=None, scratch=None):
    _chk(v, 'v'); _chk(g, 'g')
    co, ci, k = v.shape
    if out is None:
        out = torch.empty((k, ci, co), device=v.device, dtype=torch.float32)
    if scratch is None:
        scratch = torch.empty((co,), device=v.device, dtype=torch.float32)
    _hip.check(_hip.load().v2w_wn_fold_conv(v.data_ptr(), _hip.ptr(g), out.data_ptr(), scratch.data_ptr(),
                                            co, ci, k, _stream(v)), 'v2w_wn_fold_conv')
    return out


def fold_convt_weight(v, g, out=None, scratch=None):
    _chk(v, 'v'); _chk(g, 'g')
    ci, co, k = v.shape
    if out is None:
        out = torch.empty((k, ci, co), device=v.device, dtype=torch.float32)
    if scratch is None:
        scratch = torch.empty((ci,), device=v.device, dtype=torch.float32)
    _hip.check(_hip.load().v2w_wn_fold_convt(v.data_ptr(), _hip.ptr(g), out.data_ptr(), scratch.data_ptr(),
                                             ci, co, k, _stream(v)), 'v2w_wn_fold_convt')
    return out


def transpose_flip(wf, out=None):
    k, ci, co = wf.shape
    if out is None:
        out = torch.empty((k, co, ci), device=wf.device, dtype=torch.float32)
    _hip.check(_hip.load().v2w_wf_transpose_flip(wf.data_ptr(), out.data_ptr(), k, ci, co, _stream(wf)), 'v2w_wf_transpose_flip')
    return out


def gather_transpose(wf, t_start, t_step, n, out=None):
    k, ci, co = wf.shape
    if out is None:
        out = torch.empty((n, co, ci), device=wf.device, dtype=torch.float32)
    _hip.check(_hip.load().v2w_wf_gather_transpose(wf.data_ptr(), out.data_ptr(), k, ci, co, t_start, t_step, n, _stream(wf)),
               'v2w_wf_gather_transpose')
    return out


def pack_mfma(wf, out=None, u=1):
    k, ci, co = wf.shape
    if out is None:
        out = torch.empty((k * ci * co,), device=wf.device, dtype=torch.float32)
    rc = _hip.load().v2w_pack_mfma(wf.data_ptr(), out.data_ptr(), k, ci, co, u, _stream(wf))
    if rc == -2:
        return None
    _hip.check(rc, 'v2w_pack_mfma')
    return out


def pack_mfma_dgrad(wf):
    k, ci, co = wf.shape
    out = torch.empty((k * ci * co,), device=wf.device, dtype=torch.float32)
    rc = _hip.load().v2w_pack_mfma_dgrad(wf.data_ptr(), out.data_ptr(), k, co, ci, _stream(wf))
    if rc == -2:
        return None
    _hip.check(rc, 'v2w_pack_mfma_dgrad')
    return out


def pack_mfma_batch(w4):
    _chk(w4, 'w4')
    n, k, ci, co = w4.shape
    out = torch.empty((n, k * ci * co), device=w4.device, dtype=torch.float32)
    _hip.check(_hip.load().v2w_pack_mfma_batch(w4.data_ptr(), out.data_ptr(), k, ci, co, 1, n, _stream(w4)), 'v2w_pack_mfma_batch')
    return out


def split_supported(c_in, c_out, u=1):
    return bool(_hip.load().v2w_split_supported(c_in, c_out, u))


def split_halves(k, c_in, c_out):
    return k * c_in * ((c_out + 31) // 32 * 32) * 2 + 1024


def split_packable(c_in, c_out):
    return bool(_hip.load().v2w_split_packable(c_in, c_out))


def split_units_halves(k, c_in, c_out):
    return k * c_in * ((c_out + 31) // 32 * 32) * 2


def pack_split(wf, out=None, sc=None, bf16=False):
    k, ci, co = wf.shape
    if out is None:
        out = torch.empty((split_halves(k, ci, co),), device=wf.device, dtype=torch.float16)
    if sc is None:
        sc = torch.empty((4,), device=wf.device, dtype=torch.float32)
    fn = _hip.load().v2w_pack_bf16 if bf16 else _hip.load().v2w_pack_split
    _hip.check(fn(wf.data_ptr(), out.data_ptr(), sc.data_ptr(), k, ci, co, _stream(wf)), 'v2w_pack_bf16' if bf16 else 'v2w_pack_split')
    return out, sc


def _conv1d_args(a, x, wf, bias, out, *, k, dil=1, slope=1.0, in_affine=None, res=None, res_affine=None,
                 accumulate=False, out_div=0.0, algo=ALGO_AUTO, wp=None, add=None, mask=None, mask_slope=1.0,
                 in_stride=0, in_phase=0, pad_left=-1, L=None, wps=None, out_slope=0.0, group=None, io_bf16=0, rowsum=None, in_ct=0):
    B, ci, Lx = x.shape
    L = Lx if L is None else L
    co = out.shape[1]
    a.out_slope = out_slope
    a.rowsum_part = _hip.ptr(rowsum)
    a.io_bf16 = io_bf16
    xoff = ooff = 0
    if group is not None:
        g, cig, cog = group
        a.in_ct, a.out_ct = ci, co
        xoff, ooff = g * cig * Lx * 4, g * cog * out.shape[2] * 4
        ci, co = cig, cog
    if in_ct:
        a.in_ct = in_ct
    a.in_stride, a.in_phase, a.pad_left = in_stride, in_phase, pad_left
    a.in_ = x.data_ptr() + xoff
    a.in_a, a.in_s = (_hip.ptr(in_affine[0]), _hip.ptr(in_affine[1])) if in_affine is not None else (None, None)
    a.wf = _hip.ptr(wf); a.wp = _hip.ptr(wp); a.bias = _hip.ptr(bias)
    if wps is not None:
        a.wps, a.winv = wps[0].data_ptr(), wps[1].data_ptr()
    a.res = _hip.ptr(res)
    a.res_a, a.res_s = (_hip.ptr(res_affine[0]), _hip.ptr(res_affine[1])) if res_affine is not None else (None, None)
    add = list(add or [])
    a.add0 = _hip.ptr(add[0]) if len(add) > 0 else None
    a.add1 = _hip.ptr(add[1]) if len(add) > 1 else None
    if mask is not None:
        a.mask_src = mask[0].data_ptr()
        a.mask_a, a.mask_s = (mask[1][0].data_ptr(), mask[1][1].data_ptr()) if mask[1] is not None else (None, None)
    a.mask_slope = mask_slope
    a.out = out.data_ptr() + ooff
    a.B, a.C_in, a.C_out, a.L, a.k, a.dil = B, ci, co, L, k, dil
    a.slope = slope; a.accumulate = int(accumulate); a.out_div = out_div; a.algo = algo


class SplitKSlab:

    def __init__(self):
        self.t = None
        self.retired = []

    def ensure(self, nbytes, device):
        if self.t is None or self.t.device != device or self.t.numel() * 4 < nbytes:
            if self.t is not None:
                self.retired.append(self.t)
            self.t = torch.empty(((nbytes + 3) // 4,), device=device, dtype=torch.float32)
        return self.t


def _attach_slab(a, slab, nbytes, device):
    if slab is not None and nbytes > 0:
        t = slab.ensure(int(nbytes), device)
        a.splitk_ws, a.splitk_ws_bytes = t.data_ptr(), t.numel() * 4


_SPLITK_BYTES = {}


def _splitk_bytes(a, n):
    qs = [a[i] for i in range(n)] if n > 1 else [a]
    key = (n,) + tuple((q.B, q.C_in, q.C_out, q.L, q.k, q.dil, q.algo, q.accumulate, q.in_stride, q.pad_left, q.in_ct, q.out_ct, q.io_bf16,
                        bool(q.res), bool(q.add0), bool(q.add1), bool(q.mask_src), bool(q.in_a), bool(q.rowsum_part), bool(q.wps), bool(q.wp),
                        q.out_div != 0.0, q.out_slope != 0.0) for q in qs)
    v = _SPLITK_BYTES.get(key)
    if v is None:
        v = _SPLITK_BYTES[key] = int(_hip.load().v2w_conv1d_splitk_ws_bytes(a if n > 1 else C.byref(a), n))
    return v


def conv1d(x, wf, bias, out, splitk_ws=None, **kw):
    a = _hip.Conv1dArgs()
    _conv1d_args(a, x, wf, bias, out, **kw)
    if splitk_ws is not None:
        _attach_slab(a, splitk_ws, _splitk_bytes(a, 1), x.device)
    _hip.check(_hip.load().v2w_conv1d_fwd(C.byref(a), _stream(x)), 'v2w_conv1d_fwd')
    return out


def conv1d_multi(problems, splitk_ws=None):
    n = len(problems)
    if 1 < n <= 4:
        arr = (_hip.Conv1dArgs * n)()
        for a, (x, wf, bias, out, kw) in zip(arr, problems):
            _conv1d_args(a, x, wf, bias, out, **kw)
        if splitk_ws is not None:
            _attach_slab(arr[0], splitk_ws, _splitk_bytes(arr, n), problems[0][0].device)
        rc = _hip.load().v2w_conv1d_fwd_multi(arr, n, _stream(problems[0][0]))
        if rc == 0:
            return
        if rc != -2:
            _hip.check(rc, 'v2w_conv1d_fwd_multi')
    for x, wf, bias, out, kw in problems:
        conv1d(x, wf, bias, out, splitk_ws=splitk_ws, **kw)


def convt1d(x, wf, bias, out, *, k, u, slope=1.0, algo=ALGO_AUTO, wp=None, stats_part=None, splitk_ws=None):
    B, ci, L = x.shape
    a = _hip.ConvT1dArgs()
    a.in_ = x.data_ptr(); a.wf = _hip.ptr(wf); a.wp = _hip.ptr(wp); a.bias = _hip.ptr(bias); a.out = out.data_ptr()
    a.stats_part = _hip.ptr(stats_part)
    a.B, a.C_in, a.C_out, a.L, a.k, a.u = B, ci, out.shape[1], L, k, u
    a.slope = slope; a.algo = algo
    if splitk_ws is not None:
        _attach_slab(a, splitk_ws, _hip.load().v2w_convt1d_splitk_ws_bytes(C.byref(a)), x.device)
    _hip.check(_hip.load().v2w_convt1d_fwd(C.byref(a), _stream(x)), 'v2w_convt1d_fwd')
    return out


def pack_bf16_convt(wf, u, out=None):
    k, ci, co = wf.shape
    nbytes = int(_hip.load().v2w_pack_bf16_convt_bytes(k, ci, co, u))
    if nbytes == 0:
        return None
    if out is None or out.numel() * out.element_size() < nbytes:
        out = torch.empty((nbytes // 2,), device=wf.device, dtype=torch.bfloat16)
    _hip.check(_hip.load().v2w_pack_bf16_convt(wf.data_ptr(), out.data_ptr(), k, ci, co, u, _stream(wf)), 'v2w_pack_bf16_convt')
    return out


def _convt_bf16_args(x, wps, bias, out, k, u, slope, stats_part, io_bf16=0):
    B, ci, L = x.shape
    a = _hip.ConvT1dArgs()
    a.in_ = x.data_ptr(); a.wf = None; a.wp = _hip.ptr(wps); a.bias = _hip.ptr(bias); a.out = _hip.ptr(out)
    a.stats_part = _hip.ptr(stats_part)
    a.B, a.C_in, a.C_out, a.L, a.k, a.u = B, ci, out.shape[1], L, k, u
    a.slope = slope; a.algo = ALGO_BF16; a.io_bf16 = io_bf16
    return a


def convt_bf16_stats_tiles(x, out, k, u, io_bf16=0):
    n = _hip.load().v2w_convt1d_bf16_tiles(C.byref(_convt_bf16_args(x, None, None, out, k, u, 1.0, None, io_bf16)))
    return n if n > 0 else 0


def convt1d_bf16(x, wps, bias, out, *, k, u, slope=1.0, stats_part=None, io_bf16=0):
    _hip.check(_hip.load().v2w_convt1d_bf16_fwd(C.byref(_convt_bf16_args(x, wps, bias, out, k, u, slope, stats_part, io_bf16)), _stream(x)),
               'v2w_convt1d_bf16_fwd')
    return out


def cond_gamma_beta(spk, noise, fc_w: Sequence, fc_b: Sequence, sn_w: Sequence, sn_b: Sequence,
                    sn_u: Sequence, sn_v: Sequence, gb: Sequence, z_ws, sigma_ws, training: bool):
    n = len(fc_w)
    if n > _hip.V2W_MAX_STAGES:
        raise ValueError(f'at most {_hip.V2W_MAX_STAGES} upsample stages are supported')
    a = _hip.CondArgs()
    a.spk = spk.data_ptr(); a.noise = noise.data_ptr()
    for i in range(n):
        a.fc_w[i] = fc_w[i].data_ptr(); a.fc_b[i] = fc_b[i].data_ptr()
        a.sn_w[i] = sn_w[i].data_ptr(); a.sn_b[i] = sn_b[i].data_ptr()
        a.sn_u[i] = sn_u[i].data_ptr(); a.sn_v[i] = sn_v[i].data_ptr()
        a.gb[i] = gb[i].data_ptr()
        a.C[i] = sn_w[i].shape[0] // 2
    a.z_ws = z_ws.data_ptr(); a.sigma_ws = sigma_ws.data_ptr()
    a.n_stages = n; a.B = spk.shape[0]; a.spk_dim = spk.shape[1]; a.noise_dim = noise.shape[1]
    a.training = int(training)
    _hip.check(_hip.load().v2w_cond_gamma_beta(C.byref(a), _stream(spk)), 'v2w_cond_gamma_beta')


def _cond_args(a, spk, noise, fc_w, fc_b, sn_w, sn_b, sn_u, sn_v, sigma_ws):
    n = len(sn_w)
    if n > _hip.V2W_MAX_STAGES:
        raise ValueError(f'at most {_hip.V2W_MAX_STAGES} upsample stages are supported')
    a.spk = _hip.ptr(spk); a.noise = _hip.ptr(noise)
    for i in range(n):
        a.fc_w[i] = _hip.ptr(fc_w[i]) if fc_w is not None else None
        a.fc_b[i] = _hip.ptr(fc_b[i]) if fc_b is not None else None
        a.sn_w[i] = sn_w[i].data_ptr(); a.sn_b[i] = _hip.ptr(sn_b[i]) if sn_b is not None else None
        a.sn_u[i] = _hip.ptr(sn_u[i]) if sn_u is not None else None
        a.sn_v[i] = _hip.ptr(sn_v[i]) if sn_v is not None else None
        a.C[i] = sn_w[i].shape[0] // 2
    a.sigma_ws = sigma_ws.data_ptr()
    a.n_stages = n
    if spk is not None:
        a.B = spk.shape[0]; a.spk_dim = spk.shape[1]; a.noise_dim = noise.shape[1]


def cond_sigma(sn_w: Sequence, sn_u: Sequence, sn_v: Sequence, sigma_ws, training: bool = False):
    a = _hip.CondArgs()
    _cond_args(a, None, None, None, None, sn_w, None, sn_u, sn_v, sigma_ws)
    a.training = int(training)
    _hip.check(_hip.load().v2w_cond_sigma(C.byref(a), _stream(sigma_ws)), 'v2w_cond_sigma')


def cond_affine_eval(spk, noise, fc_w: Sequence, fc_b: Sequence, sn_w: Sequence, sn_b: Sequence, sigma_ws,
                     running_mean: Sequence, running_var: Sequence, eps: Sequence, a_out: Sequence, s_out: Sequence):
    e = _hip.CondEvalArgs()
    _cond_args(e.c, spk, noise, fc_w, fc_b, sn_w, sn_b, None, None, sigma_ws)
    for i in range(len(sn_w)):
        e.running_mean[i] = running_mean[i].data_ptr(); e.running_var[i] = running_var[i].data_ptr()
        e.a_out[i] = a_out[i].data_ptr(); e.s_out[i] = s_out[i].data_ptr()
        e.eps[i] = eps[i]
    _hip.check(_hip.load().v2w_cond_affine_eval(C.byref(e), _stream(spk)), 'v2w_cond_affine_eval')


def bn_stats(x, stats, partial_ws):
    B, Cc, L = x.shape
    _hip.check(_hip.load().v2w_bn_stats(x.data_ptr(), stats.data_ptr(), partial_ws.data_ptr(), B, Cc, L, _stream(x)),
               'v2w_bn_stats')
    return stats


def bn_finalize(stats, gb, running_mean, running_var, num_batches_tracked, a_out, s_out, *, training: bool,
                momentum=0.1, eps=1e-5):
    B, C2 = gb.shape
    _hip.check(_hip.load().v2w_bn_finalize(_hip.ptr(stats), gb.data_ptr(), running_mean.data_ptr(), running_var.data_ptr(),
                                           _hip.ptr(num_batches_tracked), a_out.data_ptr(), s_out.data_ptr(),
                                           B, C2 // 2, int(training), momentum, eps, _stream(gb)), 'v2w_bn_finalize')


BN_SLICES = 128


def bn_reduce_finalize_slices(part, ntiles, count, slices, gb, running_mean, running_var, num_batches_tracked, a_out, s_out, *,
                              momentum=0.1, eps=1e-5):
    B, C2 = gb.shape
    Cc = C2 // 2
    lib, st = _hip.load(), _stream(part)
    _hip.check(lib.v2w_bn_reduce_slices(part.data_ptr(), ntiles, Cc, slices.data_ptr(), BN_SLICES, st), 'v2w_bn_reduce_slices')
    _hip.check(lib.v2w_bn_finalize_slices(slices.data_ptr(), BN_SLICES, float(count), gb.data_ptr(), running_mean.data_ptr(),
                                          running_var.data_ptr(), _hip.ptr(num_batches_tracked), a_out.data_ptr(), s_out.data_ptr(),
                                          B, Cc, momentum, eps, st), 'v2w_bn_finalize_slices')


def affine_apply(x, a, s, out):
    B, Cc, L = x.shape
    _hip.check(_hip.load().v2w_affine_apply(x.data_ptr(), a.data_ptr(), s.data_ptr(), out.data_ptr(), B, Cc, L, _stream(x)),
               'v2w_affine_apply')
    return out


def conv_post_tanh(x, wf, bias, out, *, k, slope):
    B, ci, L = x.shape
    if x.dtype == torch.bfloat16:
        _hip.check(_hip.load().v2w_conv_post_tanh_bf16in(x.data_ptr(), wf.data_ptr(), _hip.ptr(bias), out.data_ptr(),
                                                         B, ci, L, k, slope, _stream(x)), 'v2w_conv_post_tanh_bf16in')
        return out
    _hip.check(_hip.load().v2w_conv_post_tanh(x.data_ptr(), wf.data_ptr(), _hip.ptr(bias), out.data_ptr(),
                                              B, ci, L, k, slope, _stream(x)), 'v2w_conv_post_tanh')
    return out


def conv_tile_config(B, c_in, c_out, L, k, dil=1, u=1, prefix=False):
    cfg = (C.c_int32 * 10)()
    if u == 1:
        a = _hip.Conv1dArgs(); a.B, a.C_in, a.C_out, a.L, a.k, a.dil = B, c_in, c_out, L, k, dil
        a.pad_left = -1
        rc = _hip.load().v2w_conv1d_tile_config(C.byref(a), cfg)
    else:
        a = _hip.ConvT1dArgs(); a.B, a.C_in, a.C_out, a.L, a.k, a.u = B, c_in, c_out, L, k, u
        rc = _hip.load().v2w_convt1d_tile_config(C.byref(a), cfg)
    if rc != 0:
        return None
    pre = 'conv_tile_kernel<' + ', '.join(str(v) for v in cfg[:9]) + ', 0, '
    return pre if prefix else pre + ('true>' if L % 4 == 0 else 'false>')


def conv_bf16_config(B, nprob, c_in, c_out, L, k, dil=1, u=1, io_bf16=3):
    cfg = (C.c_int32 * 10)()
    if u == 1:
        arr = (_hip.Conv1dArgs * nprob)()
        for a in arr:
            a.B, a.C_in, a.C_out, a.L, a.k, a.dil = B, c_in, c_out, L, k, dil
            a.pad_left = -1
            a.io_bf16 = io_bf16
        rc = _hip.load().v2w_conv1d_bf16_config(arr, nprob, cfg)
    else:
        a = _hip.ConvT1dArgs(); a.B, a.C_in, a.C_out, a.L, a.k, a.u = B, c_in, c_out, L, k, u
        a.io_bf16 = io_bf16
        a.slope = 0.1
        rc = _hip.load().v2w_convt1d_bf16_config(C.byref(a), cfg)
    if rc != 0:
        return None
    v = list(cfg)
    if v[5] == 102:
        return 'convt_bf16_res_kernel<' + ', '.join(str(x) for x in v[:5]) + f', {v[9]}>'
    tf = lambda b: 'true' if b else 'false'
    return 'conv_bf16_kernel<' + ', '.join(str(x) for x in v[:6]) + f', {tf(v[6])}, {tf(v[7])}, {v[8]}, {tf(v[9])}>'


def conv_rowsum_tiles(B, nprob, c_in, c_out, L, k, dil=1):
    cfg = (C.c_int32 * 10)()
    a = _hip.Conv1dArgs(); a.B, a.C_in, a.C_out, a.L, a.k, a.dil = B * nprob, c_in, c_out, L, k, dil
    a.pad_left = -1
    if _hip.load().v2w_conv1d_tile_config(C.byref(a), cfg) != 0:
        return 0
    return cfg[9] // nprob


def convt_stats_tiles(B, c_in, c_out, L, k, u):
    cfg = (C.c_int32 * 10)()
    a = _hip.ConvT1dArgs(); a.B, a.C_in, a.C_out, a.L, a.k, a.u = B, c_in, c_out, L, k, u
    return int(cfg[9]) if _hip.load().v2w_convt1d_tile_config(C.byref(a), cfg) == 0 else 0


def bn_reduce_partials(part, ntiles, Cc, count, stats):
    _hip.check(_hip.load().v2w_bn_reduce_partials(part.data_ptr(), ntiles, Cc, float(count), stats.data_ptr(), _stream(part)),
               'v2w_bn_reduce_partials')
    return stats


def bn_reduce_finalize(part, ntiles, count, stats, gb, running_mean, running_var, num_batches_tracked, a_out, s_out, *, momentum=0.1, eps=1e-5):
    B, C2 = gb.shape
    _hip.check(_hip.load().v2w_bn_reduce_finalize(part.data_ptr(), ntiles, float(count), gb.data_ptr(), running_mean.data_ptr(),
                                                  running_var.data_ptr(), _hip.ptr(num_batches_tracked), stats.data_ptr(), a_out.data_ptr(),
                                                  s_out.data_ptr(), B, C2 // 2, momentum, eps, _stream(gb)), 'v2w_bn_reduce_finalize')
    return a_out, s_out


class FoldPlan:

    def __init__(self, layers, device):
        n = len(layers)
        self.n = n
        layers = [tuple(l) + (None,) * (10 - len(l)) for l in layers]
        rows = [(l[3] if l[7] else l[4]) for l in layers]
        self.scale = torch.empty((sum(rows),), device=device, dtype=torch.float32)
        descs = (_hip.FoldDesc * n)()
        off = 0
        for d, (v, g, wp, ci, co, k, u, tr, wf, wpd), r in zip(descs, layers, rows):
            d.v = v.data_ptr(); d.g = _hip.ptr(g); d.wp = wp.data_ptr()
            d.wf = _hip.ptr(wf); d.wpd = _hip.ptr(wpd)
            d.scale = self.scale.data_ptr() + 4 * off
            d.c_in, d.c_out, d.k, d.u, d.transposed = ci, co, k, u, int(tr)
            off += r
        starts = (C.c_int32 * (2 * (n + 1)))()
        lds = _hip.load().v2w_fold_plan(descs, n, starts)
        _hip.check(0 if lds > 0 else (lds or -1), 'v2w_fold_plan')
        self.lds = lds
        self.nblk_scale, self.nblk_pack = starts[n], starts[2 * n + 1]
        self.descs_dev = torch.frombuffer(bytearray(bytes(descs)), dtype=torch.uint8).to(device)
        self.starts_dev = torch.tensor(list(starts), dtype=torch.int32, device=device)
        self.key = tuple((v.data_ptr(), 0 if g is None else g.data_ptr(), wp.data_ptr()) for (v, g, wp, *_r) in layers)

    def run(self):
        _hip.check(_hip.load().v2w_fold_pack_batch(self.descs_dev.data_ptr(), self.starts_dev.data_ptr(), self.n,
                                                   self.nblk_scale, self.nblk_pack, self.lds,
                                                   torch.cuda.current_stream(self.scale.device).cuda_stream),
                   'v2w_fold_pack_batch')


class SplitPlan:

    def __init__(self, layers, device, bf16=False):
        n = len(layers)
        self.n = n
        self.bf16 = bool(bf16)
        self.rowscale = torch.empty((sum(v.shape[0] for v, *_ in layers),), device=device, dtype=torch.float32)
        descs = (_hip.SplitDesc * n)()
        starts = [0] * (2 * (n + 1))
        off = blocks = 0
        for i, (d, (v, g, wps, sc)) in enumerate(zip(descs, layers)):
            co, ci, k = v.shape
            d.v = v.data_ptr(); d.g = _hip.ptr(g); d.wps = wps.data_ptr(); d.sc = sc.data_ptr()
            d.rowscale = self.rowscale.data_ptr() + 4 * off
            d.c_in, d.c_out, d.k, d.mode = ci, co, k, int(bf16)
            starts[i], starts[n + 1 + i] = off, blocks
            off += co
            blocks += ((co + 31) // 32) * (ci // 16)
        starts[n], starts[2 * n + 1] = off, blocks
        self.nblk_rows, self.nblk_pack = off, blocks
        self.k_max = max(v.shape[2] for v, *_ in layers)
        self.descs_dev = torch.frombuffer(bytearray(bytes(descs)), dtype=torch.uint8).to(device)
        self.starts_dev = torch.tensor(starts, dtype=torch.int32, device=device)
        self.key = tuple((v.data_ptr(), 0 if g is None else g.data_ptr(), w.data_ptr()) for (v, g, w, _s) in layers)

    def run(self):
        _hip.check(_hip.load().v2w_split_pack_batch(self.descs_dev.data_ptr(), self.starts_dev.data_ptr(), self.n,
                                                    self.nblk_rows, self.nblk_pack, self.k_max, int(self.bf16),
                                                    torch.cuda.current_stream(self.rowscale.device).cuda_stream),
                   'v2w_split_pack_batch')


def resblock_pair_multi(problems):
    n = len(problems)
    arr = (_hip.PairArgs * n)()
    for a, q in zip(arr, problems):
        x = q['x']
        B, Cc, L = x.shape
        a.in_ = x.data_ptr()
        aff = q.get('in_affine')
        a.in_a, a.in_s = (aff[0].data_ptr(), aff[1].data_ptr()) if aff is not None else (None, None)
        a.wp1 = q['wp1'].data_ptr(); a.bias1 = _hip.ptr(q['b1']); a.wp2 = q['wp2'].data_ptr(); a.bias2 = _hip.ptr(q['b2'])
        add = list(q.get('add') or [])
        a.add0 = _hip.ptr(add[0]) if len(add) > 0 else None
        a.add1 = _hip.ptr(add[1]) if len(add) > 1 else None
        a.out = q['out'].data_ptr()
        a.B, a.C, a.L, a.k, a.dil1, a.dil2 = B, Cc, L, q['k'], q['dil1'], q['dil2']
        a.res_mode = q['res_mode']; a.slope = q['slope']; a.out_div = q.get('out_div', 0.0)
    rc = _hip.load().v2w_resblock_pair_fwd(arr, n, _stream(problems[0]['x']))
    if rc == -2:
        return False
    _hip.check(rc, 'v2w_resblock_pair_fwd')
    return True


def resblock1_pairs_ok(B, Cc, L, ks, dil1s, dil2s, *, slope) -> bool:
    a = _hip.StageSplitArgs()
    a.rb1 = 1
    for j, (k, d1, d2) in enumerate(zip(ks, dil1s, dil2s)):
        a.k[j], a.dil1[j], a.dil2[j] = k, d1, d2
    a.nk, a.B, a.C, a.L = len(ks), B, Cc, L
    a.slope, a.out_div, a.bf16, a.io_bf16 = slope, 0.0, 1, 3
    return _hip.load().v2w_resblock2_stage_split_config(C.byref(a)) == 0


def resblock2_stage_split_ok(B, Cc, L, ks, dil1s, dil2s, *, slope, bf16=True, io_bf16=3) -> bool:
    a = _hip.StageSplitArgs()
    for j, (k, d1, d2) in enumerate(zip(ks, dil1s, dil2s)):
        a.k[j], a.dil1[j], a.dil2[j] = k, d1, d2
    a.nk, a.B, a.C, a.L = len(ks), B, Cc, L
    a.slope, a.out_div, a.bf16, a.io_bf16 = slope, float(len(ks)), int(bf16), io_bf16
    return _hip.load().v2w_resblock2_stage_split_config(C.byref(a)) == 0


def resblock2_stage_up_tiles(B, Cc, L, ks, dil1s, dil2s, *, slope, up_k, up_u, up_slope) -> int:
    a = _hip.StageSplitArgs()
    for j, (k, d1, d2) in enumerate(zip(ks, dil1s, dil2s)):
        a.k[j], a.dil1[j], a.dil2[j] = k, d1, d2
    a.nk, a.B, a.C, a.L = len(ks), B, Cc, L
    a.slope, a.out_div, a.bf16, a.io_bf16 = slope, float(len(ks)), 1, 3
    a.up_k, a.up_u, a.up_slope = up_k, up_u, up_slope
    n = _hip.load().v2w_resblock2_stage_up_tiles(C.byref(a))
    return n if n > 0 else 0


def resblock1_pairs_bf16(ins, in_affine, branches, outs, *, slope, out_div=0.0, add=None):
    B, Cc, L = ins[0].shape
    a = _hip.StageSplitArgs()
    a.rb1 = 1
    a.in_a, a.in_s = (in_affine[0].data_ptr(), in_affine[1].data_ptr()) if in_affine is not None else (None, None)
    for j, q in enumerate(branches):
        a.wps1[j], a.sc1[j], a.bias1[j] = q['wps1'][0].data_ptr(), q['wps1'][1].data_ptr(), _hip.ptr(q['b1'])
        a.wps2[j], a.sc2[j], a.bias2[j] = q['wps2'][0].data_ptr(), q['wps2'][1].data_ptr(), _hip.ptr(q['b2'])
        a.k[j], a.dil1[j], a.dil2[j] = q['k'], q['dil1'], q['dil2']
        a.in_b[j] = ins[j].data_ptr(); a.out_b[j] = outs[j].data_ptr()
    add = list(add or [])
    a.add0 = _hip.ptr(add[0]) if len(add) > 0 else None
    a.add1 = _hip.ptr(add[1]) if len(add) > 1 else None
    a.nk, a.B, a.C, a.L = len(branches), B, Cc, L
    a.slope, a.out_div, a.bf16, a.io_bf16 = slope, out_div, 1, 3
    rc = _hip.load().v2w_resblock2_stage_split_fwd(C.byref(a), _stream(ins[0]))
    if rc == -2:
        return False
    _hip.check(rc, 'v2w_resblock2_stage_split_fwd (rb1)')
    return True


def resblock2_stage_split(x, in_affine, branches, out, *, slope, out_div, bf16=False, io_bf16=0, post=None, up=None):
    B, Cc, L = x.shape
    a = _hip.StageSplitArgs()
    if up is not None:
        a.up_wps, a.up_bias, a.up_out, a.up_stats_part = up[0].data_ptr(), _hip.ptr(up[1]), up[2].data_ptr(), _hip.ptr(up[3])
        a.up_k, a.up_u, a.up_slope = up[4], up[5], up[6]
    a.in_ = x.data_ptr()
    a.in_a, a.in_s = (in_affine[0].data_ptr(), in_affine[1].data_ptr()) if in_affine is not None else (None, None)
    for j, q in enumerate(branches):
        a.wps1[j], a.sc1[j], a.bias1[j] = q['wps1'][0].data_ptr(), q['wps1'][1].data_ptr(), _hip.ptr(q['b1'])
        a.wps2[j], a.sc2[j], a.bias2[j] = q['wps2'][0].data_ptr(), q['wps2'][1].data_ptr(), _hip.ptr(q['b2'])
        a.k[j], a.dil1[j], a.dil2[j] = q['k'], q['dil1'], q['dil2']
    a.out = _hip.ptr(out)
    a.nk, a.B, a.C, a.L = len(branches), B, Cc, L
    a.slope, a.out_div, a.bf16 = slope, out_div, int(bf16)
    a.io_bf16 = io_bf16
    if post is not None:
        a.post_w, a.post_b, a.post_out = post[0].data_ptr(), _hip.ptr(post[1]), post[2].data_ptr()
        a.post_k, a.post_slope = post[3], post[4]
    rc = _hip.load().v2w_resblock2_stage_split_fwd(C.byref(a), _stream(x))
    if rc == -2:
        return False
    _hip.check(rc, 'v2w_resblock2_stage_split_fwd')
    return True


def branch_convs_bf16(mode, ins, in_affine, wps, biases, outs, ks, dils, *, slope, out_div=0.0):
# ... 202 lines not shown
```

wavthruvec_pytorch_amd/models.py:

```python
from __future__ import annotations

import math
import warnings
from typing import Dict, List, Optional

import contextlib
import torch
import torch.nn as nn

from . import _hip, hipops
from .modules import ConditionalBatchNorm1d
from .utils import get_padding, init_weights

LRELU_SLOPE = 0.1
_SIDE_STREAMS: Dict[str, 'torch.cuda.Stream'] = {}
_CAPTURE_STREAMS: Dict[str, 'torch.cuda.Stream'] = {}
_Z_CHANNEL = 128


class _WNConvBase(nn.Module):
    transposed = False

    def __init__(self, in_channels, out_channels, kernel_size, stride=1, dilation=1, padding=0):
        super().__init__()
# ... 8 lines not shown
        self.weight_v = nn.Parameter(v)

    @property
    def weight_normed(self) -> bool:
        return 'weight_g' in self._parameters

    def remove_weight_norm(self):
        if not self.weight_normed:
            raise ValueError(f'weight_norm of \'weight\' not found in {self}')
        with torch.no_grad():
            v, g = self.weight_v, self.weight_g
            w = v * (g / v.flatten(1).norm(dim=1).view(-1, 1, 1))
        del self._parameters['weight_g']
        del self._parameters['weight_v']
        self.weight = nn.Parameter(w.detach())

    def extra_repr(self):
        s = f'{self.in_channels}, {self.out_channels}, kernel_size=({self.kernel_size},), stride=({self.stride},)'
        if self.padding:
            s += f', padding=({self.padding},)'
        if self.dilation != 1:
            s += f', dilation=({self.dilation},)'
        return s


class Conv1d(_WNConvBase):
    transposed = False


class ConvTranspose1d(_WNConvBase):
    transposed = True


def _fold_one(m, device):
    v, g = (m.weight_v.detach(), m.weight_g.detach()) if m.weight_normed else (m.weight.detach(), None)
    wf = hipops.fold_conv_weight(v, g)
    return wf, hipops.pack_mfma(wf)


def _resblock_forward(rb, x, pairs):
    if not x.is_cuda:
        raise RuntimeError('ResBlock (HIP): GPU tensors only; there is no CPU fallback')
    if torch.is_grad_enabled() and (x.requires_grad or any(p.requires_grad for p in rb.parameters())):
        from .backward import ResBlockFunction
        names, params = zip(*rb.named_parameters())
        return ResBlockFunction.apply(rb, pairs, names, x, *params)
    with torch.no_grad():
        cur = x.detach().contiguous().float()
        for ca, cb in pairs:
            wfa, wpa = _fold_one(ca, cur.device)
            if cb is None:
                out = torch.empty_like(cur)
                hipops.conv1d(cur, wfa, ca.bias.detach(), out, k=ca.kernel_size, dil=ca.dilation, slope=LRELU_SLOPE, res=cur, wp=wpa)
            else:
                t = torch.empty_like(cur)
                hipops.conv1d(cur, wfa, ca.bias.detach(), t, k=ca.kernel_size, dil=ca.dilation, slope=LRELU_SLOPE, wp=wpa)
                wfb, wpb = _fold_one(cb, cur.device)
                out = torch.empty_like(cur)
                hipops.conv1d(t, wfb, cb.bias.detach(), out, k=cb.kernel_size, dil=cb.dilation, slope=LRELU_SLOPE, res=cur, wp=wpb)
            cur = out
        return cur


class ResBlock1(nn.Module):

    def __init__(self, h, channels, kernel_size=3, dilation=(1, 3, 5)):
        super().__init__()
        self.h = h
        self.channels, self.kernel_size, self.dilation = channels, kernel_size, tuple(dilation)
        self.convs1 = nn.ModuleList([
            Conv1d(channels, channels, kernel_size, 1, dilation=d, padding=get_padding(kernel_size, d))
            for d in dilation[:3]])
        self.convs2 = nn.ModuleList([
            Conv1d(channels, channels, kernel_size, 1, dilation=1, padding=get_padding(kernel_size, 1))
            for _ in range(3)])

    @_hip.on_tensor_device
    def forward(self, x):
        return _resblock_forward(self, x, [(c1, c2) for c1, c2 in zip(self.convs1, self.convs2)])

    def remove_weight_norm(self):
        for l in self.convs1:
            l.remove_weight_norm()
        for l in self.convs2:
            l.remove_weight_norm()


class ResBlock2(nn.Module):

    def __init__(self, h, channels, kernel_size=3, dilation=(1, 3)):
        super().__init__()
        self.h = h
        self.channels, self.kernel_size, self.dilation = channels, kernel_size, tuple(dilation)
        self.convs = nn.ModuleList([
            Conv1d(channels, channels, kernel_size, 1, dilation=d, padding=get_padding(kernel_size, d))
            for d in dilation[:2]])

    @_hip.on_tensor_device
    def forward(self, x):
        return _resblock_forward(self, x, [(c, None) for c in self.convs])

    def remove_weight_norm(self):
        for l in self.convs:
            l.remove_weight_norm()


class Generator(nn.Module):

    def __init__(self, h):
        super().__init__()
        self.h = h
        self.num_kernels = len(h.resblock_kernel_sizes)
        self.num_upsamples = len(h.upsample_rates)
        if self.num_upsamples > 8:
            raise ValueError('at most 8 upsample stages are supported')
        c0 = h.upsample_initial_channel
        self.conv_pre = Conv1d(h.num_wv_feat, c0, 7, 1, padding=3)
        resblock = ResBlock1 if h.resblock == '1' else ResBlock2

        self.ups = nn.ModuleList()
        for i, (u, k) in enumerate(zip(h.upsample_rates, h.upsample_kernel_sizes)):
            self.ups.append(ConvTranspose1d(c0 // (2 ** i), c0 // (2 ** (i + 1)), k, u, padding=(k - u) // 2))

        self.resblocks = nn.ModuleList()
        ch = c0
        for i in range(len(self.ups)):
            ch = c0 // (2 ** (i + 1))
            for j, (k, d) in enumerate(zip(h.resblock_kernel_sizes, h.resblock_dilation_sizes)):
                self.resblocks.append(resblock(h, ch, k, d))

        self.conv_post = Conv1d(ch, 1, 7, 1, padding=3)

        self.cbns = nn.ModuleList()
        self.fcs = nn.ModuleList()
        for i in range(len(self.ups)):
            self.fcs.append(nn.Linear(h.spk_dim + h.noise_dim, _Z_CHANNEL))
            self.cbns.append(ConditionalBatchNorm1d(256 // pow(2, i)))
            if self.cbns[i].num_features != self.ups[i].out_channels:
                raise ValueError('ConditionalBatchNorm1d widths are 256 // 2**i (models.py:113): '
                                 'upsample_initial_channel must be 512')

        self.algo = hipops.ALGO_AUTO
        self.stat_sync = None
        self.always_refold = True
        self.fuse_pairs = (16,)
        self.fuse_stage = (8, 16, 32)
        self.precision = 'f32'
        self.split_min_channels = 64
        self.bf16_storage = True
        self.fuse_wide = True
        self.fuse_wide_stage = True
        self.fuse_up = True
        self.fuse_bn_finalize = True
        self.merge_waits = True
        self.cond_stream = None
        self.fuse_post = True
        self.fuse_stage_backward = False
        self._split_wide = set()
        self._ws: Dict[str, torch.Tensor] = {}
        self._slabs: Dict[tuple, 'hipops.SplitKSlab'] = {}
        self._wts: Dict[str, torch.Tensor] = {}
        self._fold_key: Dict[str, tuple] = {}
        self._profile = None
        self._profile_names = None
        self.use_launch_plan = True
        self._tapes: Dict[tuple, object] = {}
        self._ws_epoch = 0
        self._tape_refused = 0

    def __getstate__(self):
        st = self.__dict__.copy()
        st.update(_tapes={}, _ws={}, _slabs={}, _wts={}, _fold_key={}, _profile=None, _profile_names=None, _ws_epoch=0)
        return st

    def enable_sync_batchnorm(self, group=None, single_rank_collective=None):
        from .distributed import BNStatSync
        self.stat_sync = BNStatSync(group, single_rank_collective=single_rank_collective)
        return self

    def profile_kernel_names(self, x, spk_emb, noise):
        keep = self._profile
        self._profile, self._profile_names = [], {}
        try:
            with torch.no_grad():
                self.forward(x, spk_emb, noise)
            return dict(self._profile_names)
        finally:
            self._profile, self._profile_names = keep, None

    def capture_graph(self, x, spk_emb, noise, warmup: int = 2):
        if self.stat_sync is not None:
            raise RuntimeError('capture_graph: the RCCL statistics all-reduce cannot be part of a captured graph')
        sx, ss, sn = x.detach().clone().contiguous(), spk_emb.detach().clone().contiguous(), noise.detach().clone().contiguous()
        with torch.no_grad():
            side = _CAPTURE_STREAMS.get(str(sx.device))
            if side is None:
                side = _CAPTURE_STREAMS[str(sx.device)] = torch.cuda.Stream(device=sx.device)
            side.wait_stream(torch.cuda.current_stream(sx.device))
            with torch.cuda.stream(side):
                for _ in range(max(1, warmup)):
                    self.forward(sx, ss, sn)
            torch.cuda.current_stream(sx.device).wait_stream(side)
            graph = torch.cuda.CUDAGraph()
            with torch.cuda.graph(graph, stream=side):
                sy = self.forward(sx, ss, sn)

        epoch = self._ws_epoch

        def run(x, spk_emb, noise):
            if self._ws_epoch != epoch:
                raise RuntimeError('capture_graph: the module reallocated its buffers since this graph was captured (a forward of another '
                                   'configuration ran): capture again - a module serves one captured configuration at a time')
            if x.dtype == sx.dtype and spk_emb.dtype == ss.dtype and noise.dtype == sn.dtype and x.device == sx.device:
                torch._foreach_copy_([sx, ss, sn], [x, spk_emb, noise])
            else:
                sx.copy_(x); ss.copy_(spk_emb); sn.copy_(noise)
            graph.replay()
            return sy

        run.graph = graph
        return run

    def remove_weight_norm(self):
        print('Removing weight norm...')
        for l in self.ups:
            l.remove_weight_norm()
        for l in self.resblocks:
            l.remove_weight_norm()
        self.conv_pre.remove_weight_norm()
        self.conv_post.remove_weight_norm()

    @staticmethod
    def _side_stream(device, index=0):
        key = str(device) if index == 0 else f'{device}#{index}'
        st = _SIDE_STREAMS.get(key)
        if st is None:
            st = _SIDE_STREAMS[key] = torch.cuda.Stream(device=device)
        return st

    def _buf(self, name, shape, dtype=torch.float32, device=None):
        t = self._ws.get(name)
        if t is None or tuple(t.shape) != tuple(shape) or t.dtype != dtype or t.device != device:
            if t is not None:
                self._drop_tapes()
            t = torch.empty(shape, device=device, dtype=dtype)
            self._ws[name] = t
        return t

    def _drop_tapes(self):
        self._ws_epoch += 1
        self._tapes.clear()

    def _slab(self, device):
        key = (str(device), torch.cuda.current_stream(device).cuda_stream)
        slab = self._slabs.get(key)
        if slab is None:
            if len(self._slabs) >= 16:
                self._slabs.pop(next(iter(self._slabs)))
                self._drop_tapes()
            slab = self._slabs[key] = hipops.SplitKSlab()
        return slab

    def _wbuf(self, name, shape, dtype=torch.float32, device=None):
        t = self._wts.get(name)
        if t is None or tuple(t.shape) != tuple(shape) or t.dtype != dtype or t.device != device:
            if t is not None:
                self._drop_tapes()
            t = torch.empty(shape, device=device, dtype=dtype)
            self._wts[name] = t
        return t

    def _conv_layers(self):
        yield 'conv_pre', self.conv_pre
        for i, m in enumerate(self.ups):
            yield f'ups.{i}', m
        for i, rb in enumerate(self.resblocks):
            if isinstance(rb, ResBlock1):
                for n, m in enumerate(rb.convs1):
                    yield f'resblocks.{i}.convs1.{n}', m
                for n, m in enumerate(rb.convs2):
                    yield f'resblocks.{i}.convs2.{n}', m
            else:
                for n, m in enumerate(rb.convs):
                    yield f'resblocks.{i}.convs.{n}', m
        yield 'conv_post', self.conv_post

    def invalidate_weight_cache(self):
        self._fold_key.clear()

    def _fold_weights(self, device, need_wf=False, bf16_only=False):
        layers = list(self._conv_layers())
        vers = []
        for name, m in layers:
            ps = (m.weight_v, m.weight_g) if m.weight_normed else (m.weight,)
            vers.append(tuple((p.data_ptr(), p._version) for p in ps))
        state = (tuple(vers), self.algo, str(device), need_wf, bf16_only)
        force = (self.training and self.always_refold) or need_wf
        if not force and self._fold_key.get('state') == state:
            return self._fold_key['wf'], self._fold_key['wp']
        wf, wp, batch = {}, {}, []
        wpd = {}
        for name, m in layers:
            if bf16_only and name != 'conv_post':
                wf[name], wp[name] = None, None
                continue
            v, g = (m.weight_v.detach(), m.weight_g.detach()) if m.weight_normed else (m.weight.detach(), None)
            u = m.stride if m.transposed else 1
            mfma_ok = (self.algo != hipops.ALGO_DIRECT and name != 'conv_post' and
                       hipops.conv_tile_config(1, m.in_channels, m.out_channels, 64, m.kernel_size,
                                               1 if m.transposed else m.dilation, u) is not None)
            if mfma_ok and need_wf:
                n_el = m.kernel_size * m.in_channels * m.out_channels
                wfb = self._wbuf('wf.' + name, (m.kernel_size, m.in_channels, m.out_channels), device=device)
                wpb = self._wbuf('wp.' + name, (n_el,), device=device)
                wdb = None
                if not m.transposed and m.in_channels == m.out_channels and name.startswith('resblocks.'):
                    wdb = wpd[name] = self._wbuf('wpd.' + name, (n_el,), device=device)
                batch.append((v, g, wpb, m.in_channels, m.out_channels, m.kernel_size, u, m.transposed, wfb, wdb))
                wf[name], wp[name] = wfb, wpb
            elif mfma_ok:
                wpb = self._wbuf('wp.' + name, (m.kernel_size * m.in_channels * m.out_channels,), device=device)
                batch.append((v, g, wpb, m.in_channels, m.out_channels, m.kernel_size, u, m.transposed))
                wf[name], wp[name] = None, wpb
            else:
                wfb = self._wbuf('wf.' + name, (m.kernel_size, m.in_channels, m.out_channels), device=device)
                scratch = self._wbuf('wf_scratch', (max(2048, m.out_channels, m.in_channels),), device=device)
                (hipops.fold_convt_weight if m.transposed else hipops.fold_conv_weight)(v, g, wfb, scratch)
                wf[name], wp[name] = wfb, None
        if batch:
            key = tuple((q[0].data_ptr(), 0 if q[1] is None else q[1].data_ptr(), q[2].data_ptr(),
                         0 if len(q) < 9 or q[8] is None else q[8].data_ptr()) for q in batch)
            plan = self._fold_key.get('plan')
            if plan is None or plan.key != key:
                self._drop_tapes()
                plan = hipops.FoldPlan(batch, device)
                plan.key = key
                self._fold_key['plan'] = plan
            plan.run()
        self._fold_key.update(state=state, wf=wf, wp=wp, wpd=wpd, vers=tuple(vers), gen=self._fold_key.get('gen', 0) + 1)
        return wf, wp

    def _split_weights(self, device, all_ups=False, ups_stream=None, mark=None, between=None):
        if self.precision == 'f32' or self.algo == hipops.ALGO_DIRECT:
            return {}
        if self.precision not in ('f16x3', 'bf16'):
            raise ValueError(f"Generator.precision must be 'f32', 'f16x3' or 'bf16', got {self.precision!r}")
        gen = (self._fold_key.get('gen', 0), self.precision, all_ups)
        cached = self._fold_key.get('wps')
        if cached is not None and cached[0] == gen:
            return cached[1]
        out, batch = {}, []
        self._split_wide = set()
        picked = []
        for name, m in self._conv_layers():
            if m.transposed or name == 'conv_post':
                continue
            stage32 = (m.in_channels == m.out_channels and m.out_channels in (16, 32) and m.out_channels in self.fuse_stage
                       and name.startswith('resblocks.') and ('.convs.' in name or (all_ups and self.precision == 'bf16')))
            wide = (m.out_channels >= self.split_min_channels and hipops.split_supported(m.in_channels, m.out_channels)
                    and m.kernel_size % 2 == 1 and m.kernel_size >= 3)
            if wide or stage32:
                picked.append((name, m, wide))
        sizes = [hipops.split_halves(m.kernel_size, m.in_channels, m.out_channels) if wide
                 else hipops.split_units_halves(m.kernel_size, m.in_channels, m.out_channels) for _n, m, wide in picked]
        arena = self._buf('wps.arena', (sum(sizes) + 1024,), dtype=torch.float16, device=device)
        scs = self._buf('wsc.arena', (4 * max(1, len(picked)),), device=device)
        off = 0
        for i, ((name, m, wide), n) in enumerate(zip(picked, sizes)):
            v, g = (m.weight_v.detach(), m.weight_g.detach()) if m.weight_normed else (m.weight.detach(), None)
            wpsb, scb = arena[off:off + n], scs[4 * i:4 * i + 4]
            off += n
            batch.append((v.contiguous(), g, wpsb, scb))
            out[name] = (wpsb, scb)
            if wide:
                self._split_wide.add(name)
        first = [q for (nm, _m, _w), q in zip(picked, batch) if nm == 'conv_pre'] if ups_stream is not None else batch
        rest = [q for (nm, _m, _w), q in zip(picked, batch) if nm != 'conv_pre'] if ups_stream is not None else []
        if mark is None or ups_stream is None:
            def mark(name):
                pass

        def run_plan(slot, sub, strm):
            if not sub:
                return
            key = tuple((v.data_ptr(), 0 if g is None else g.data_ptr(), w.data_ptr()) for (v, g, w, _s) in sub) + (self.precision,)
            plan = self._fold_key.get(slot)
            if plan is None or plan.key != key:
                self._drop_tapes()
                plan = hipops.SplitPlan(sub, device, bf16=self.precision == 'bf16')
                plan.key = key
                self._fold_key[slot] = plan
            with (torch.cuda.stream(strm) if strm is not None else contextlib.nullcontext()):
                plan.run()

        def fold_up(i, m):
            v, g = (m.weight_v.detach(), m.weight_g.detach()) if m.weight_normed else (m.weight.detach(), None)
            wfb = self._buf(f'wfbf.ups.{i}', (m.kernel_size, m.in_channels, m.out_channels), device=device)
            scratch = self._buf('wf_scratch_ups', (max(2048, m.out_channels, m.in_channels),), device=device)
            with (torch.cuda.stream(ups_stream) if ups_stream is not None else contextlib.nullcontext()):
                hipops.fold_convt_weight(v, g, wfb, scratch)
                w = hipops.pack_bf16_convt(wfb, m.stride, out=self._ws.get(f'wpsbf.ups.{i}'))
            if w is not None:
                if self._ws.get(f'wpsbf.ups.{i}') is not w:
                    self._drop_tapes()
                self._ws[f'wpsbf.ups.{i}'] = w
                out[f'ups.{i}'] = w
            if i == 0:
                mark(f'ups.{i}')

        ups_bf = [(i, m) for i, m in enumerate(self.ups) if self.precision == 'bf16' and (m.out_channels >= 64 or all_ups)]
        run_plan('split_plan', first, None)
        if ups_bf and ups_bf[0][0] == 0:
            fold_up(*ups_bf.pop(0))
        if between is not None:
            between()
        for i, m in ups_bf:
            fold_up(i, m)
        run_plan('split_plan_rest', rest, ups_stream)
        mark('rest')
        self._fold_key['wps'] = (gen, out)
        return out

    def _bf16_storage_kernels_exist(self, B, T) -> bool:
        key = (B, T, self.num_kernels, tuple(self.fuse_stage))
        hit = self._fold_key.get('bf16_storage_ok')
        if hit is not None and hit[0] == key:
            return hit[1]
        ok = hipops.conv_bf16_config(B, 1, self.conv_pre.in_channels, self.conv_pre.out_channels, T, 7, 1, 1, io_bf16=2) is not None
        L, nk = T, self.num_kernels
        for i, up in enumerate(self.ups):
            ok = ok and hipops.conv_bf16_config(B, 1, up.in_channels, up.out_channels, L, up.kernel_size, 1, up.stride, io_bf16=3) is not None
            L *= up.stride
            C = up.out_channels
            rbs = self.resblocks[i * nk:(i + 1) * nk]
            if isinstance(rbs[0], ResBlock1):
                for n in range(3):
                    pair = hipops.resblock1_pairs_ok(B, C, L, [rb.kernel_size for rb in rbs], [rb.convs1[n].dilation for rb in rbs],
                                                     [1] * len(rbs), slope=LRELU_SLOPE)
                    convs = C >= 64 and all(rb.kernel_size >= 3 and
                                            hipops.conv_bf16_config(B, 1, C, C, L, rb.kernel_size, rb.convs1[n].dilation, 1, io_bf16=3) is not None and
                                            hipops.conv_bf16_config(B, 1, C, C, L, rb.kernel_size, 1, 1, io_bf16=3) is not None for rb in rbs)
                    ok = ok and all(rb.kernel_size % 2 == 1 for rb in rbs) and (pair or convs)
            elif C in (16, 32):
                ok = ok and all(rb.kernel_size % 2 == 1 for rb in rbs) and hipops.resblock2_stage_split_ok(
                    B, C, L, [rb.kernel_size for rb in rbs], [rb.convs[0].dilation for rb in rbs], [rb.convs[1].dilation for rb in rbs],
                    slope=LRELU_SLOPE)
            else:
                for rb in rbs:
                    for c in rb.convs:
                        ok = ok and rb.kernel_size % 2 == 1 and rb.kernel_size >= 3 and \
                            hipops.conv_bf16_config(B, 1, C, C, L, rb.kernel_size, c.dilation, 1, io_bf16=3) is not None
        self._fold_key['bf16_storage_ok'] = (key, bool(ok))
        return bool(ok)

    @_hip.on_tensor_device
    def forward(self, x, spk_emb=None, noise=None):
        if spk_emb is None or noise is None:
            raise TypeError('Generator.forward: spk_emb and noise are required')
        if not (x.is_cuda and spk_emb.is_cuda and noise.is_cuda):
            raise RuntimeError('Generator.forward runs on the MI355X HIP path only: move inputs and module to a GPU '
                               '(there is no CPU/PyTorch fallback)')
        dev = x.device
        if self.conv_pre.bias.device != dev:
            raise RuntimeError(f'Generator parameters live on {self.conv_pre.bias.device}, inputs on {dev}')
        if x.dim() != 3 or x.shape[1] != self.h.num_wv_feat:
            raise RuntimeError(f'expected x of shape (B, {self.h.num_wv_feat}, T), got {tuple(x.shape)}')
        needs_grad = torch.is_grad_enabled() and (x.requires_grad or any(p.requires_grad for p in self.parameters()))
        x_in = x.contiguous().float()
        x = x_in.detach()
        spk = spk_emb.detach().contiguous().float()
        nz = noise.detach().contiguous().float()
        if spk.shape != (x.shape[0], self.h.spk_dim) or nz.shape != (x.shape[0], self.h.noise_dim):
            raise RuntimeError('spk_emb / noise must be (B, spk_dim) / (B, noise_dim)')
        if needs_grad:
            if self.algo == hipops.ALGO_DIRECT:
                raise NotImplementedError('Generator (HIP): the scalar cross-check kernels (algo = ALGO_DIRECT) serve no-grad forwards only; '
                                          'back-propagation needs the MFMA schedule (algo = ALGO_AUTO)')
            from .backward import GeneratorFunction
            names, params = zip(*[(n, q) for n, q in self.named_parameters()])
            return GeneratorFunction.apply(self, names, x_in if x_in.requires_grad else x, spk, nz, *params)
        return self._forward_hip(x, spk, nz, None)

    def _plan_key(self, x):
        ptrs = tuple(p.data_ptr() for p in self.parameters()) + tuple(b.data_ptr() for b in self.buffers())
        return (tuple(x.shape), str(x.device), torch.cuda.current_stream(x.device).cuda_stream, self.training, self.precision, self.algo, self.bf16_storage, tuple(self.fuse_stage), tuple(self.fuse_pairs),
                self.fuse_wide, self.fuse_wide_stage, self.fuse_up, self.fuse_post, self.fuse_bn_finalize, self.cond_stream, self.merge_waits, self.split_min_channels,
                self.always_refold, ptrs)

    def _forward_hip(self, x, spk, nz, save):
        from .forward_plan import ForwardPlanner, DirectStreams
        from . import schedule
        dev = x.device
        main, side, side2 = torch.cuda.current_stream(dev), self._side_stream(dev), self._side_stream(dev, 1)
        if save is not None or not self.use_launch_plan or self.stat_sync is not None:
            return ForwardPlanner(self, x, spk, nz, save, DirectStreams(main, side, side2)).run()
        key, refold = self._tape_key(x)
        tape = self._tapes.get(key)
        if tape is not None:
            y = torch.empty(tape.out[0], device=dev, dtype=tape.out[1])
            tape.replay(main, side, dict(x=x.data_ptr(), spk=spk.data_ptr(), nz=nz.data_ptr(), y=y.data_ptr()), self._profile, side2)
            if self._profile_names is not None:
                self._profile_names.update(tape.kernel_names())
            if refold is not None:
                wvers, sigma = refold
                if wvers is not None:
                    self._fold_key['gen'] = self._fold_key.get('gen', 0) + 1
                    if wvers:
                        self._fold_key.update(vers=wvers, state=(wvers,) + tape.fold_state_tail)
                if sigma:
                    self._fold_key['sigma'] = self._sigma_key(dev)
            if self.training:
                self._fold_key.pop('sigma', None)
            return y
        if self._profile is not None:
            return ForwardPlanner(self, x, spk, nz, None, DirectStreams(main, side, side2)).run()
        rec = schedule.Recorder(_hip.load(), main, side, side2)
        epoch = self._ws_epoch
        prev = _hip.set_recorder(rec)
        try:
            y = ForwardPlanner(self, x, spk, nz, None, rec).run()
        finally:
            _hip.set_recorder(prev)
        binds = dict(x=x.data_ptr(), spk=spk.data_ptr(), nz=nz.data_ptr(), y=y.data_ptr())
        if self._ws_epoch != epoch:
            self._tapes.clear()
        state = self._fold_key.get('state')
        if len(set(binds.values())) == 4 and state is not None:
            try:
                rec.tape.finalize(binds, owned=self._owned_ranges())
            except schedule.TapeNotOwned:
                self._tape_refused += 1
                return y
            rec.tape.out = (tuple(y.shape), y.dtype)
            rec.tape.fold_state_tail = tuple(state[1:])
            self._tapes[key] = rec.tape
        return y

    def _owned_ranges(self):
        from . import schedule
        ts = list(self.parameters()) + list(self.buffers()) + list(self._ws.values()) + list(self._wts.values())
        for slab in self._slabs.values():
            ts += [slab.t] + list(slab.retired)
        ts += list(schedule.tensors_in(self._fold_key))
        return schedule.owned_ranges(ts)

    def _sigma_key(self, dev):
        sn_p = [q for c in self.cbns for q in (c.layer.weight_orig, c.layer.weight_u, c.layer.weight_v)]
        return (tuple((q.data_ptr(), q._version) for q in sn_p), str(dev))

    def _tape_key(self, x):
        base = self._plan_key(x)
        if self.training and self.always_refold:
            return base + ('refold',), ((), False)
        vers = self._param_versions()
        wstale = not (self._fold_key.get('vers') == vers and self._fold_key.get('state') is not None)
        sstale = (not self.training) and self._fold_key.get('sigma') != self._sigma_key(x.device)
        if not (wstale or sstale):
            return base + ('folded',), None
        return base + (('w' if wstale else '') + ('s' if sstale else ''),), (vers if wstale else None, sstale)

    def _param_versions(self):
        vers = []
        for _name, m in self._conv_layers():
            ps = (m.weight_v, m.weight_g) if m.weight_normed else (m.weight,)
            vers.append(tuple((p.data_ptr(), p._version) for p in ps))
        return tuple(vers)
```

Before: 307.9 million samples/s.

## Add Winograd F(2,3) MFMA conv1d path for f32 dilated convolutions

Adds a Winograd-style minimal-filtering conv1d kernel that splits each kernel into 3-tap segments and computes two outputs per position with four MFMA products instead of six. Pre-transformed weights are packed during the weight-fold pass, and eligible f32 layers (channels multiple of 32/64, non-transposed) are routed to the new kernel by default. This cuts the matrix-multiply work for the k=3/5/7 resblock convs. In exchange it adds input transform arithmetic, extra packed weight buffers, and possible f32 rounding differences.

```diff
diff --git a/include/vec2wav_hip.h b/include/vec2wav_hip.h
--- a/include/vec2wav_hip.h
+++ b/include/vec2wav_hip.h
@@ -7,7 +7,7 @@
 extern "C" {
 #endif
 
-#define V2W_ABI_VERSION 34
+#define V2W_ABI_VERSION 35
 
 #define V2W_E_ARG      (-1)
 #define V2W_E_SHAPE    (-2)
@@ -18,6 +18,7 @@
 #define V2W_ALGO_MFMA   2
 #define V2W_ALGO_BF16   4
 #define V2W_ALGO_SPLIT  3
+#define V2W_ALGO_WINO   5
 
 int         v2w_abi_version(void);
 const char* v2w_build_arch(void);
@@ -37,6 +38,8 @@
 int v2w_pack_mfma(const float* wf, float* wp, int k, int c_in, int c_out, int u, void* stream);
 int v2w_pack_mfma_dgrad(const float* wf, float* wp, int k, int c_in, int c_out, void* stream);
 int v2w_pack_mfma_batch(const float* wf, float* wp, int k, int c_in, int c_out, int u, int n, void* stream);
+int v2w_pack_wino(const float* wf, float* wpw, int k, int c_in, int c_out, void* stream);
+int v2w_wino_terms(int k);
 
 typedef struct {
     const float* v; const float* g; float* wp; float* scale;
@@ -45,6 +48,7 @@
     int32_t _pad;
     float* wf;
     float* wpd;
+    float* wpw;
 } v2w_fold_desc;
 int v2w_fold_plan(v2w_fold_desc* descs, int n, int32_t* starts);
 int v2w_fold_pack_batch(const v2w_fold_desc* descs_dev, const int32_t* starts_dev, int n,
diff --git a/wavthruvec_pytorch_amd/_hip.py b/wavthruvec_pytorch_amd/_hip.py
--- a/wavthruvec_pytorch_amd/_hip.py
+++ b/wavthruvec_pytorch_amd/_hip.py
@@ -6,10 +6,10 @@
 
 from . import build as _build
 
-ABI_VERSION = 34
+ABI_VERSION = 35
 V2W_MAX_STAGES = 8
 V2W_BN_SPLITS = 64
-ALGO_AUTO, ALGO_DIRECT, ALGO_MFMA, ALGO_SPLIT, ALGO_BF16 = 0, 1, 2, 3, 4
+ALGO_AUTO, ALGO_DIRECT, ALGO_MFMA, ALGO_SPLIT, ALGO_BF16, ALGO_WINO = 0, 1, 2, 3, 4, 5
 
 _fp = C.c_void_p
 
@@ -54,7 +54,7 @@
 class FoldDesc(C.Structure):
     _fields_ = [('v', _fp), ('g', _fp), ('wp', _fp), ('scale', _fp),
                 ('c_in', C.c_int32), ('c_out', C.c_int32), ('k', C.c_int32), ('u', C.c_int32), ('transposed', C.c_int32),
-                ('mf', C.c_int32), ('ck', C.c_int32), ('_pad', C.c_int32), ('wf', _fp), ('wpd', _fp)]
+                ('mf', C.c_int32), ('ck', C.c_int32), ('_pad', C.c_int32), ('wf', _fp), ('wpd', _fp), ('wpw', _fp)]
 
 
 _P4 = _fp * 4
@@ -111,6 +111,8 @@
     'v2w_pack_mfma': (C.c_int, [_fp, _fp, C.c_int, C.c_int, C.c_int, C.c_int, _fp]),
     'v2w_pack_mfma_batch': (C.c_int, [_fp, _fp, C.c_int, C.c_int, C.c_int, C.c_int, C.c_int, _fp]),
     'v2w_pack_mfma_dgrad': (C.c_int, [_fp, _fp, C.c_int, C.c_int, C.c_int, _fp]),
+    'v2w_pack_wino': (C.c_int, [_fp, _fp, C.c_int, C.c_int, C.c_int, _fp]),
+    'v2w_wino_terms': (C.c_int, [C.c_int]),
     'v2w_split_supported': (C.c_int, [C.c_int, C.c_int, C.c_int]),
     'v2w_pack_split': (C.c_int, [_fp, _fp, _fp, C.c_int, C.c_int, C.c_int, _fp]),
     'v2w_mel_phases': (C.c_int, [_fp, _fp, C.c_int, C.c_int, C.c_int, C.c_int, C.c_int, _fp]),
diff --git a/wavthruvec_pytorch_amd/build.py b/wavthruvec_pytorch_amd/build.py
--- a/wavthruvec_pytorch_amd/build.py
+++ b/wavthruvec_pytorch_amd/build.py
@@ -13,8 +13,8 @@
 OBJ_DIR = os.path.join(CSRC, '_obj')
 LIB_PATH = os.path.join(PKG_DIR, 'libvec2wav_hip.so')
 SOURCES = ['v2w_api.hip', 'v2w_conv_mfma.hip', 'v2w_conv_split.hip', 'v2w_conv_bf16.hip', 'v2w_conv_bf16_res.hip', 'v2w_convt_bf16_res.hip', 'v2w_stage_split.hip', 'v2w_stage_bf16.hip', 'v2w_stage_bf16_wide.hip', 'v2w_stage_bf16_n16.hip', 'v2w_stage_bf16_n16s.hip', 'v2w_stage_bf16_n32s.hip', 'v2w_resblock_fused.hip', 'v2w_stage_small.hip',
-           'v2w_wgrad.hip', 'v2w_wgrad_bf16.hip', 'v2w_backward.hip', 'v2w_direct.hip', 'v2w_conv_post_bf16.hip', 'v2w_cbn.hip', 'v2w_fold.hip', 'v2w_mel.hip', 'v2w_disc.hip']
-HEADERS = ['v2w_common.h', 'v2w_tile.h', os.path.join('..', '..', 'include', 'vec2wav_hip.h')]
+           'v2w_wgrad.hip', 'v2w_wgrad_bf16.hip', 'v2w_backward.hip', 'v2w_direct.hip', 'v2w_conv_post_bf16.hip', 'v2w_cbn.hip', 'v2w_fold.hip', 'v2w_mel.hip', 'v2w_disc.hip', 'v2w_conv_wino.hip']
+HEADERS = ['v2w_common.h', 'v2w_tile.h', 'v2w_wino.h', os.path.join('..', '..', 'include', 'vec2wav_hip.h')]
 FLAGS = ['--offload-arch=gfx950', '-O3', '-std=c++17', '-fPIC']
 
 
diff --git a/wavthruvec_pytorch_amd/csrc/v2w_api.hip b/wavthruvec_pytorch_amd/csrc/v2w_api.hip
--- a/wavthruvec_pytorch_amd/csrc/v2w_api.hip
+++ b/wavthruvec_pytorch_amd/csrc/v2w_api.hip
@@ -4,6 +4,7 @@
 int v2w_convt1d_mfma(const v2w_convt1d_args* a, hipStream_t stream, int* cfg_out, long long* ws_query = nullptr);
 int v2w_conv1d_split(const v2w_conv1d_args* a, int n, hipStream_t stream, bool bf16);
 int v2w_conv1d_direct(const v2w_conv1d_args* a, hipStream_t stream);
+int v2w_conv1d_wino(const v2w_conv1d_args* a, int n, hipStream_t stream);
 int v2w_convt1d_direct(const v2w_convt1d_args* a, hipStream_t stream);
 
 extern "C" int v2w_abi_version(void) { return V2W_ABI_VERSION; }
@@ -43,6 +44,7 @@
         case V2W_ALGO_MFMA: return v2w_conv1d_mfma(a, 1, st, nullptr);
         case V2W_ALGO_SPLIT: return v2w_conv1d_split(a, 1, st, false);
         case V2W_ALGO_BF16: return v2w_conv1d_split(a, 1, st, true);
+        case V2W_ALGO_WINO: return v2w_conv1d_wino(a, 1, st);
         case V2W_ALGO_AUTO: {
             const int rc = v2w_conv1d_mfma(a, 1, st, nullptr);
             return rc == V2W_E_SHAPE ? (a->wf ? v2w_conv1d_direct(a, st) : V2W_E_ARG) : rc;
@@ -96,5 +98,6 @@
     }
     if (a[0].algo == V2W_ALGO_SPLIT || a[0].algo == V2W_ALGO_BF16)
         return v2w_conv1d_split(a, n, (hipStream_t)stream, a[0].algo == V2W_ALGO_BF16);
+    if (a[0].algo == V2W_ALGO_WINO) return v2w_conv1d_wino(a, n, (hipStream_t)stream);
     return v2w_conv1d_mfma(a, n, (hipStream_t)stream, nullptr);
 }
diff --git a/wavthruvec_pytorch_amd/csrc/v2w_conv_mfma.hip b/wavthruvec_pytorch_amd/csrc/v2w_conv_mfma.hip
--- a/wavthruvec_pytorch_amd/csrc/v2w_conv_mfma.hip
+++ b/wavthruvec_pytorch_amd/csrc/v2w_conv_mfma.hip
@@ -1,5 +1,6 @@
 #include <type_traits>
 #include "v2w_tile.h"
+#include "v2w_wino.h"
 
 #ifdef V2W_TIMELINE
 V2W_TL_SETTER(v2w_timeline_set_tile)
@@ -781,6 +782,18 @@
         }
         const int c = gg * CKG + j * KSTEP + lane / MF, co = lane % MF;
         dst[o] = d.transposed ? tile[c * rstride + co * K + t] : tile[co * rstride + c * K + t];
+    }
+    if (d.wpw) {
+        const int nfr = wino_terms(K) * GPC;
+        float* dw = d.wpw + (size_t)(mb * nch + ch) * nfr * 256;
+        for (int o = threadIdx.x; o < nfr * 256; o += 256) {
+            const int j = o & 3, lane = (o >> 2) & 63;
+            int s0, ntap, gg, term;
+            wino_frag(K, GPC, o >> 8, s0, ntap, gg, term);
+            const int c = gg * CKG + j * KSTEP + lane / MF, co = lane % MF;
+            const float* w = tile + co * rstride + c * K + s0;
+            dw[o] = wino_weight(ntap, term, w[0], ntap > 1 ? w[1] : 0.f, ntap > 2 ? w[2] : 0.f);
+        }
     }
     if (d.wf) {
         for (int idx = threadIdx.x; idx < K * CK * MF; idx += 256) {
@@ -935,6 +948,7 @@
         if (!cfg.mf) return V2W_E_SHAPE;
         d.mf = cfg.mf; d.ck = cfg.ck;
         if (d.wpd && (d.transposed || d.c_in != d.c_out || cfg.mf != cfg.ck)) return V2W_E_ARG;
+        if (d.wpw && (d.transposed || cfg.mf != 32 || cfg.ck != 32 || wino_terms(d.k) == 0)) return V2W_E_ARG;
         starts[i] = bs; starts[n + 1 + i] = bp;
         bs += d.transposed ? d.c_in : d.c_out;
         bp += (d.c_out / cfg.mf) * (d.c_in / cfg.ck);
diff --git a/wavthruvec_pytorch_amd/csrc/v2w_conv_wino.hip b/wavthruvec_pytorch_amd/csrc/v2w_conv_wino.hip
--- /dev/null
+++ b/wavthruvec_pytorch_amd/csrc/v2w_conv_wino.hip
@@ -0,0 +1,357 @@
+#include "v2w_tile.h"
+#include "v2w_wino.h"
+
+namespace {
+
+constexpr int WCK = 32;
+constexpr int WRS = 36;
+constexpr int WGPC = 4;
+constexpr int WHMAX = 32;
+__host__ __device__ constexpr int wslot(int c) { return (c & ~7) + 4 * (c & 1) + ((c & 7) >> 1); }
+__host__ __device__ constexpr int wpair_c0(int P) { return 8 * (P >> 2) + 4 * (P & 1) + ((P >> 1) & 1); }
+__host__ __device__ inline int wino_tpos(int P, int d) { const int q = P / d; return 2 * d * q + (P - q * d); }
+
+template <int MI, int WN, int NPF, bool VEC>
+__global__ void __launch_bounds__(128 * WN, 3)
+conv_wino_kernel(const MultiArgs m) {
+    typedef Frag<32> F;
+    typedef F::acc_t acc_t;
+    constexpr int WM = 2;
+    constexpr int NTHREADS = 64 * WM * WN;
+    constexpr int MT = 32 * MI * WM;
+    constexpr int NTP = 32 * WN;
+    constexpr int RING = 4;
+
+    extern __shared__ __attribute__((aligned(16))) float smem[];
+
+    int pq = 0;
+#pragma unroll
+    for (int i = 1; i < V2W_MAX_MULTI; ++i) pq += (int)blockIdx.x >= m.start[i] ? 1 : 0;
+    const TileArgs& p = m.p[pq];
+    const int mtiles = p.Cout / MT;
+    const int id = blockIdx.x - m.start[pq];
+    const int grp = id / (8 * mtiles), rem = id % (8 * mtiles);
+    const int mt = rem >> 3;
+    const int tile = grp * 8 + (rem & 7);
+    if (tile >= p.ntiles) return;
+    const int b = tile / p.ntl;
+    const int P0 = (tile % p.ntl) * NTP;
+    const int m0 = mt * MT;
+    const int d = p.dil;
+
+    const int tid = threadIdx.x;
+    const int lane = tid & 63;
+    const int wave = __builtin_amdgcn_readfirstlane(tid >> 6);
+    const int lr = lane & 31;
+    const int hk = lane >> 5;
+    const int wm0 = (wave / WN) * (32 * MI);
+    const int wn0 = (wave % WN) * 32;
+    const int L = p.L, K = p.K;
+    const float slope = p.slope;
+    const int nch = p.Cin / WCK;
+    const int pos0 = (wino_tpos(P0, d) - p.hl) & ~3;
+    const int bufsz = p.xrows * WRS;
+    float* const etab = smem + p.atab_off;
+    float* const atab = etab + 3 * MT;
+
+    acc_t acc[4][MI];
+#pragma unroll
+    for (int c = 0; c < 4; ++c)
+#pragma unroll
+        for (int i = 0; i < MI; ++i)
+#pragma unroll
+            for (int e = 0; e < 16; ++e) acc[c][i][e] = 0.f;
+
+    const int nq = p.xrows >> 2;
+    const int nq8 = (nq + 7) >> 3;
+    const unsigned magic = (unsigned)(((1ull << 32) + nq8 - 1) / nq8);
+    f32x4 pf[NPF][2];
+    const f32x4 zero4 = {0.f, 0.f, 0.f, 0.f};
+    auto item = [&](int s, int& c0, int& row, bool& in_img, bool& in_seq) {
+        int t = tid;
+        asm volatile("" : "+v"(t));
+        const int idx = t + s * NTHREADS;
+        const int g = idx >> 4;
+        const int pg = (int)__umulhi((unsigned)g, magic);
+        const int quad = (g - pg * nq8) * 8 + (idx & 7);
+        const int P = 2 * pg + ((idx >> 3) & 1);
+        row = quad * 4;
+        in_img = quad < nq && P < WCK / 2;
+        c0 = wpair_c0(in_img ? P : 0);
+        const int pos = pos0 + row;
+        in_seq = in_img && pos >= 0 && pos < L;
+    };
+    auto prefetch = [&](int ci0) {
+        const float* src = p.in + (size_t)(b * p.CinT + ci0) * L + pos0;
+#pragma unroll
+        for (int s = 0; s < NPF; ++s) {
+            int c0, row; bool in_img, in_seq;
+            item(s, c0, row, in_img, in_seq);
+            pf[s][0] = zero4; pf[s][1] = zero4;
+            if (in_seq) {
+                pf[s][0] = *reinterpret_cast<const f32x4*>(src + (size_t)c0 * L + row);
+                pf[s][1] = *reinterpret_cast<const f32x4*>(src + (size_t)(c0 + 2) * L + row);
+            }
+        }
+    };
+    auto commit = [&](int ci0, float* Xs) {
+#pragma unroll
+        for (int s = 0; s < NPF; ++s) {
+            int c0, row; bool in_img, in_seq;
+            item(s, c0, row, in_img, in_seq);
+            if (!in_img) continue;
+            float a0 = 1.f, s0 = 0.f, a1 = 1.f, s1 = 0.f;
+            if (p.in_a) {
+                a0 = atab[ci0 + c0]; s0 = atab[p.Cin + ci0 + c0];
+                a1 = atab[ci0 + c0 + 2]; s1 = atab[p.Cin + ci0 + c0 + 2];
+            }
+            float* dst = Xs + row * WRS + wslot(c0);
+#pragma unroll
+            for (int e = 0; e < 4; ++e) {
+                f32x2 v = {0.f, 0.f};
+                if (in_seq) { v[0] = v2w_lrelu(fmaf(a0, pf[s][0][e], s0), slope); v[1] = v2w_lrelu(fmaf(a1, pf[s][1][e], s1), slope); }
+                *reinterpret_cast<f32x2*>(dst + e * WRS) = v;
+            }
+        }
+    };
+    auto stage_scalar = [&](int ci0, float* Xs) {
+        for (int c = wave; c < WCK; c += WM * WN) {
+            const int ch = b * p.CinT + ci0 + c;
+            const float* src = p.in + (size_t)ch * L;
+            const float av = p.in_a ? p.in_a[ch] : 1.f;
+            const float sv = p.in_s ? p.in_s[ch] : 0.f;
+            float* dst = Xs + wslot(c);
+            for (int j = lane; j < p.xrows; j += 64) {
+                const int l = pos0 + j;
+                float v = 0.f;
+                if (l >= 0 && l < L) v = v2w_lrelu(fmaf(av, src[l], sv), slope);
+                dst[j * WRS] = v;
+            }
+        }
+    };
+
+    const int nfrag = nch * wino_terms(K) * WGPC;
+    const f32x4* ap[MI];
+#pragma unroll
+    for (int i = 0; i < MI; ++i)
+        ap[i] = reinterpret_cast<const f32x4*>(p.wp) + ((size_t)((m0 + wm0) / 32 + i) * nfrag) * 64;
+    int fidx = 0;
+    f32x4 ar[RING][MI];
+    const unsigned lane16 = (unsigned)lane * 16u;
+    auto load_next = [&](f32x4 (&a)[MI]) {
+        const int f = fidx < nfrag ? fidx : nfrag - 1;
+        unsigned l16 = lane16;
+        asm volatile("" : "+v"(l16));
+#pragma unroll
+        for (int i = 0; i < MI; ++i)
+            a[i] = *reinterpret_cast<const f32x4*>(reinterpret_cast<const char*>(ap[i] + (size_t)f * 64) + l16);
+        ++fidx;
+    };
+
+    auto segment = [&](auto ntap_c, const float* x, int dstep) {
+        constexpr int NTAP = decltype(ntap_c)::value;
+        constexpr int NX = NTAP + 1;
+        constexpr int NTERM = wino_seg_terms(NTAP);
+#pragma unroll
+        for (int gg = 0; gg < WGPC; ++gg) {
+            f32x4 xr[NX];
+#pragma unroll
+            for (int j = 0; j < NX; ++j) xr[j] = *reinterpret_cast<const f32x4*>(x + j * dstep + 8 * gg);
+            f32x4 u[NTERM];
+            if constexpr (NTAP == 3) {
+                u[0] = xr[0] - xr[2]; u[1] = xr[1] + xr[2];
+                u[2] = xr[2] - xr[1]; u[3] = xr[1] - xr[3];
+            } else if constexpr (NTAP == 2) {
+                u[0] = xr[0] - xr[1]; u[1] = xr[1]; u[2] = xr[1] - xr[2];
+            } else {
+                u[0] = xr[0]; u[1] = xr[1];
+            }
+            __builtin_amdgcn_sched_barrier(0);
+#pragma unroll
+            for (int t = 0; t < NTERM; ++t) {
+                const int cls = NTAP == 3 ? t : (NTAP == 2 ? (t == 2 ? 3 : t) : (t == 1 ? 3 : 0));
+                const int slot = (gg * NTERM + t) % RING;
+                load_next(ar[(slot + RING - 1) % RING]);
+#pragma unroll
+                for (int kk = 0; kk < 4; ++kk)
+#pragma unroll
+                    for (int i = 0; i < MI; ++i) acc[cls][i] = F::mfma(ar[slot][i][kk], u[t][kk], acc[cls][i]);
+            }
+        }
+    };
+
+    for (int c = tid; c < MT; c += NTHREADS) {
+        etab[c] = p.bias ? p.bias[m0 + c] : 0.f;
+        etab[MT + c] = p.res_a ? p.res_a[b * p.Cout + m0 + c] : 1.f;
+        etab[2 * MT + c] = p.res_a ? p.res_s[b * p.Cout + m0 + c] : 0.f;
+    }
+    if (p.in_a) {
+        for (int c = tid; c < p.Cin; c += NTHREADS) {
+            atab[c] = p.in_a[b * p.Cin + c];
+            atab[p.Cin + c] = p.in_s[b * p.Cin + c];
+        }
+        __syncthreads();
+    }
+    if constexpr (VEC) { prefetch(0); commit(0, smem); }
+    else stage_scalar(0, smem);
+#pragma unroll
+    for (int g = 0; g + 1 < RING; ++g) load_next(ar[g]);
+    __builtin_amdgcn_sched_barrier(0);
+    __syncthreads();
+
+    const int P = P0 + wn0 + lr;
+    const int t0 = wino_tpos(P, d);
+    const int lbase = (t0 - p.hl - pos0) * WRS + 4 * hk;
+    const int dstep = d * WRS;
+    typedef std::integral_constant<int, 3> S3;
+    typedef std::integral_constant<int, 2> S2;
+    typedef std::integral_constant<int, 1> S1;
+    for (int ch = 0; ch < nch; ++ch) {
+        const float* Xs = smem + (ch & 1) * bufsz;
+        float* Xn = smem + ((ch + 1) & 1) * bufsz;
+        const bool more = ch + 1 < nch;
+        const float* xt = Xs + lbase;
+        int s = 0;
+        for (; s + 3 <= K; s += 3) segment(S3{}, xt + s * dstep, dstep);
+        if (K - s == 2) segment(S2{}, xt + s * dstep, dstep);
+        else if (K - s == 1) segment(S1{}, xt + s * dstep, dstep);
+        if (more) {
+            if constexpr (VEC) { prefetch((ch + 1) * WCK); commit((ch + 1) * WCK, Xn); }
+            else stage_scalar((ch + 1) * WCK, Xn);
+            __syncthreads();
+        }
+    }
+
+    float* const outp = p.out;
+    const float dinv = p.out_div != 0.f ? 1.f / p.out_div : 1.f;
+#pragma unroll
+    for (int i = 0; i < MI; ++i) {
+#pragma unroll
+        for (int e = 0; e < 16; ++e) {
+            const int col = wm0 + i * 32 + F::row(e, hk);
+            const float M0 = acc[0][i][e], M1 = acc[1][i][e], M2 = acc[2][i][e], M3 = acc[3][i][e];
+            const float y[2] = {(M0 + M1) + M2, (M1 - M2) - M3};
+            const size_t rowoff = ((size_t)b * p.CoutT + m0 + col) * L;
+            const float bias = etab[col], ra = etab[MT + col], rs = etab[2 * MT + col];
+#pragma unroll
+            for (int h = 0; h < 2; ++h) {
+                const int pos = t0 + h * d;
+                if (pos >= L) continue;
+                const size_t go = rowoff + pos;
+                float t = y[h] + bias;
+                if (p.res) t += fmaf(ra, p.res[go], rs);
+                if (p.add1) t += p.add0[go] + p.add1[go];
+                else if (p.accumulate) t += outp[go];
+                else if (p.add0) t += p.add0[go];
+                if (p.out_div != 0.f) t = v2w_div_by(t, p.out_div, dinv);
+                outp[go] = t;
+            }
+        }
+    }
+}
+
+template <int MI, int WN>
+int launch_wino(const TileArgs* ps, int nprob, hipStream_t stream) {
+    constexpr int MT = 64 * MI, NTP = 32 * WN, NTHREADS = 128 * WN;
+    constexpr int NPF = ((WCK / 2) * (((2 * NTP + 2 * WHMAX) / 4 + 7) / 8 * 8) + NTHREADS - 1) / NTHREADS;
+    static_assert(NTHREADS * NPF < 8 * 8192, "item index range of the magic division");
+    MultiArgs m{};
+    size_t lds = 0;
+    int grid = 0;
+    bool vec = true;
+    for (int i = 0; i < nprob; ++i) {
+        TileArgs p = ps[i];
+        if (p.Cout % MT != 0) return V2W_E_SHAPE;
+        const int d = p.dil;
+        const int npairs = d * ((p.L + 2 * d - 1) / (2 * d));
+        p.ntl = (npairs + NTP - 1) / NTP;
+        p.ntiles = p.B * p.ntl;
+        int rows = 0;
+        for (int tl = 0; tl < p.ntl; ++tl) {
+            const int P0 = tl * NTP;
+            const int pos0 = (wino_tpos(P0, d) - p.hl) & ~3;
+            const int r = wino_tpos(P0 + NTP - 1, d) + d + p.hr - pos0 + 1;
+            if (r > rows) rows = r;
+        }
+        p.xrows = (rows + 3) & ~3;
+        if (p.xrows > 2 * NTP + 2 * WHMAX) return V2W_E_SHAPE;
+        p.vec4 = (p.L % 4 == 0) && ((reinterpret_cast<uintptr_t>(p.in) & 15) == 0);
+        vec = vec && p.vec4;
+        const int nbuf = p.Cin / WCK > 1 ? 2 : 1;
+        p.atab_off = nbuf * p.xrows * WRS;
+        const size_t l = ((size_t)p.atab_off + 3 * MT + (p.in_a ? 2 * p.Cin : 0)) * sizeof(float);
+        if (l > lds) lds = l;
+        m.p[i] = p;
+        m.start[i] = grid;
+        grid += ((p.ntiles + 7) / 8) * 8 * (p.Cout / MT);
+    }
+    m.start[nprob] = grid;
+    for (int i = nprob + 1; i <= V2W_MAX_MULTI; ++i) m.start[i] = 0x7fffffff;
+    if (lds > 160 * 1024) return V2W_E_SHAPE;
+    auto kern = vec ? conv_wino_kernel<MI, WN, NPF, true> : conv_wino_kernel<MI, WN, NPF, false>;
+    if (lds > 64 * 1024) {
+        hipError_t e = v2w_max_lds(reinterpret_cast<const void*>(kern), (int)lds, stream);
+        if (e != hipSuccess) return (int)e;
+    }
+    V2W_LAUNCH(kern, dim3(grid), dim3(NTHREADS), lds, stream, m);
+    return v2w_launch_status();
+}
+
+__global__ void __launch_bounds__(256)
+pack_wino_kernel(const float* __restrict__ wf, float* __restrict__ wp, int K, int Cin, int Cout) {
+    const int nch = Cin / WCK, nfr = wino_terms(K) * WGPC;
+    const size_t total = (size_t)(Cout / 32) * nch * nfr * 256;
+    for (size_t o = (size_t)blockIdx.x * 256 + threadIdx.x; o < total; o += (size_t)gridDim.x * 256) {
+        const int j = o & 3, lane = (o >> 2) & 63;
+        size_t rest = o >> 8;
+        const int fi = rest % nfr; rest /= nfr;
+        const int ch = rest % nch;
+        const int mb = rest / nch;
+        int s0, ntap, gg, term;
+        wino_frag(K, WGPC, fi, s0, ntap, gg, term);
+        const int c = ch * WCK + gg * 8 + 2 * j + lane / 32, co = mb * 32 + lane % 32;
+        auto g = [&](int t) { return t < ntap ? wf[((size_t)(s0 + t) * Cin + c) * Cout + co] : 0.f; };
+        wp[o] = wino_weight(ntap, term, g(0), g(1), g(2));
+    }
+}
+
+}
+
+int v2w_conv1d_wino(const v2w_conv1d_args* a, int n, hipStream_t stream) {
+    if (n < 1 || n > V2W_MAX_MULTI) return V2W_E_ARG;
+    TileArgs ps[V2W_MAX_MULTI];
+    long wgs = 0;
+    const int MT = 64;
+    for (int i = 0; i < n; ++i) {
+        const v2w_conv1d_args* q = a + i;
+        if (q->B != a->B || q->C_in != a->C_in || q->C_out != a->C_out || q->L != a->L) return V2W_E_SHAPE;
+        if (q->C_in % WCK != 0 || q->C_in < 64 || q->C_out % 64 != 0 || wino_terms(q->k) == 0 || q->pad_left >= 0) return V2W_E_SHAPE;
+        if (q->in_stride > 1 || q->mask_src || q->rowsum_part || (q->out_slope != 0.f && q->out_slope != 1.f)) return V2W_E_SHAPE;
+        if ((q->in_ct > 0 && q->in_ct != q->C_in) || (q->out_ct > 0 && q->out_ct != q->C_out)) return V2W_E_SHAPE;
+        if (!q->wp) return V2W_E_ARG;
+        TileArgs p{};
+        p.in = q->in; p.in_a = q->in_a; p.in_s = q->in_s; p.wp = q->wp; p.bias = q->bias;
+        p.res = q->res; p.res_a = q->res_a; p.res_s = q->res_s; p.out = q->out;
+        p.add0 = q->add0; p.add1 = q->add1;
+        p.B = q->B; p.Cin = q->C_in; p.Cout = q->C_out; p.L = q->L; p.K = q->k; p.dil = q->dil;
+        p.CinT = q->C_in; p.CoutT = q->C_out;
+        p.hl = p.hr = q->dil * (q->k - 1) / 2;
+        p.slope = q->slope; p.accumulate = q->accumulate; p.out_div = q->out_div;
+        ps[i] = p;
+        const int npairs = q->dil * ((q->L + 2 * q->dil - 1) / (2 * q->dil));
+        wgs += (long)q->B * ((npairs + 63) / 64) * (q->C_out / MT);
+    }
+    if (wgs <= 128) return V2W_E_SHAPE;
+    return launch_wino<1, 2>(ps, n, stream);
+}
+
+extern "C" int v2w_wino_terms(int k) { return wino_terms(k); }
+
+extern "C" int v2w_pack_wino(const float* wf, float* wpw, int k, int c_in, int c_out, void* stream) {
+    if (!wf || !wpw || k <= 0 || c_in <= 0 || c_out <= 0) return V2W_E_ARG;
+    if (wino_terms(k) == 0 || c_in % WCK != 0 || c_out % 32 != 0) return V2W_E_SHAPE;
+    const size_t total = (size_t)wino_terms(k) * c_in * c_out;
+    int grid = (int)((total + 255) / 256); if (grid > 4096) grid = 4096;
+    V2W_LAUNCH(pack_wino_kernel, dim3(grid), dim3(256), 0, (hipStream_t)stream, wf, wpw, k, c_in, c_out);
+    return v2w_launch_status();
+}
diff --git a/wavthruvec_pytorch_amd/csrc/v2w_wino.h b/wavthruvec_pytorch_amd/csrc/v2w_wino.h
--- /dev/null
+++ b/wavthruvec_pytorch_amd/csrc/v2w_wino.h
@@ -0,0 +1,34 @@
+#pragma once
+
+namespace {
+
+__host__ __device__ constexpr int wino_seg_terms(int ntap) { return ntap == 3 ? 4 : (ntap == 2 ? 3 : 2); }
+__host__ __device__ constexpr int wino_terms(int k) {
+    return (k < 3 || (k & 1) == 0) ? 0 : 4 * (k / 3) + (k % 3 == 2 ? 3 : (k % 3 == 1 ? 2 : 0));
+}
+
+__host__ __device__ inline void wino_frag(int k, int gpc, int fi, int& s0, int& ntap, int& gg, int& term) {
+    s0 = 0;
+    for (;;) {
+        ntap = k - s0 >= 3 ? 3 : k - s0;
+        const int nt = wino_seg_terms(ntap);
+        if (fi < nt * gpc) { gg = fi / nt; term = fi - gg * nt; return; }
+        fi -= nt * gpc;
+        s0 += ntap;
+    }
+}
+
+__host__ __device__ inline float wino_weight(int ntap, int term, float g0, float g1, float g2) {
+    if (ntap == 3) {
+        switch (term) {
+            case 0: return g0;
+            case 1: return ((g0 + g2) + g1) * 0.5f;
+            case 2: return ((g0 + g2) - g1) * 0.5f;
+            default: return g2;
+        }
+    }
+    if (ntap == 2) return term == 0 ? g0 : (term == 1 ? g0 + g1 : g1);
+    return term == 0 ? g0 : -g0;
+}
+
+}
diff --git a/wavthruvec_pytorch_amd/forward_plan.py b/wavthruvec_pytorch_amd/forward_plan.py
--- a/wavthruvec_pytorch_amd/forward_plan.py
+++ b/wavthruvec_pytorch_amd/forward_plan.py
@@ -212,6 +212,9 @@
             return dict(algo=hipops.ALGO_BF16 if g.precision == 'bf16' else hipops.ALGO_SPLIT, wps=self.wps[nm])
         if self.st:
             raise RuntimeError(f'bf16 storage: layer {nm} has no bf16 kernel (set generator.bf16_storage = False)')
+        wpw = g._fold_key.get('wpw', {}).get(nm)
+        if wpw is not None:
+            return dict(algo=self.algo, wp=self.wp[nm], wpw=wpw)
         return dict(algo=self.algo, wp=self.wp[nm])
 
     def conv_pre(self):
diff --git a/wavthruvec_pytorch_amd/hipops.py b/wavthruvec_pytorch_amd/hipops.py
--- a/wavthruvec_pytorch_amd/hipops.py
+++ b/wavthruvec_pytorch_amd/hipops.py
@@ -7,8 +7,8 @@
 
 from . import _hip
 
-ALGO_AUTO, ALGO_DIRECT, ALGO_MFMA, ALGO_SPLIT, ALGO_BF16 = (_hip.ALGO_AUTO, _hip.ALGO_DIRECT, _hip.ALGO_MFMA, _hip.ALGO_SPLIT,
-                                                             _hip.ALGO_BF16)
+ALGO_AUTO, ALGO_DIRECT, ALGO_MFMA, ALGO_SPLIT, ALGO_BF16, ALGO_WINO = (_hip.ALGO_AUTO, _hip.ALGO_DIRECT, _hip.ALGO_MFMA, _hip.ALGO_SPLIT,
+                                                                        _hip.ALGO_BF16, _hip.ALGO_WINO)
 
 
 def _chk(t: Optional[torch.Tensor], name: str, dtype=torch.float32):
@@ -110,6 +110,24 @@
 
 def split_units_halves(k, c_in, c_out):
     return k * c_in * ((c_out + 31) // 32 * 32) * 2
+
+
+def wino_terms(k):
+    return int(_hip.load().v2w_wino_terms(k))
+
+
+def pack_wino(wf, out=None):
+    k, ci, co = wf.shape
+    n = wino_terms(k) * ci * co
+    if n == 0:
+        return None
+    if out is None:
+        out = torch.empty((n,), device=wf.device, dtype=torch.float32)
+    rc = _hip.load().v2w_pack_wino(wf.data_ptr(), out.data_ptr(), k, ci, co, _stream(wf))
+    if rc == -2:
+        return None
+    _hip.check(rc, 'v2w_pack_wino')
+    return out
 
 
 def pack_split(wf, out=None, sc=None, bf16=False):
@@ -195,6 +213,10 @@
 
 
 def conv1d(x, wf, bias, out, splitk_ws=None, **kw):
+    if kw.get('wpw') is not None:
+        conv1d_wino_multi([(x, wf, bias, out, kw)], splitk_ws=splitk_ws)
+        return out
+    kw.pop('wpw', None)
     a = _hip.Conv1dArgs()
     _conv1d_args(a, x, wf, bias, out, **kw)
     if splitk_ws is not None:
@@ -205,6 +227,9 @@
 
 def conv1d_multi(problems, splitk_ws=None):
     n = len(problems)
+    if any(kw.get('wpw') is not None for *_r, kw in problems):
+        return conv1d_wino_multi(problems, splitk_ws=splitk_ws)
+    problems = [(x, wf, bias, out, {q: v for q, v in kw.items() if q != 'wpw'}) for x, wf, bias, out, kw in problems]
     if 1 < n <= 4:
         arr = (_hip.Conv1dArgs * n)()
         for a, (x, wf, bias, out, kw) in zip(arr, problems):
@@ -218,6 +243,20 @@
             _hip.check(rc, 'v2w_conv1d_fwd_multi')
     for x, wf, bias, out, kw in problems:
         conv1d(x, wf, bias, out, splitk_ws=splitk_ws, **kw)
+
+
+def conv1d_wino_multi(problems, splitk_ws=None):
+    n = len(problems)
+    if 1 <= n <= 4 and all(kw.get('wpw') is not None for *_r, kw in problems):
+        arr = (_hip.Conv1dArgs * n)()
+        for a, (x, wf, bias, out, kw) in zip(arr, problems):
+            _conv1d_args(a, x, wf, bias, out, **{**{q: v for q, v in kw.items() if q != 'wpw'}, 'algo': ALGO_WINO, 'wp': kw['wpw']})
+        rc = _hip.load().v2w_conv1d_fwd_multi(arr, n, _stream(problems[0][0]))
+        if rc == 0:
+            return
+        if rc != -2:
+            _hip.check(rc, 'v2w_conv1d_fwd_multi')
+    conv1d_multi([(x, wf, bias, out, {q: v for q, v in kw.items() if q != 'wpw'}) for x, wf, bias, out, kw in problems], splitk_ws=splitk_ws)
 
 
 def convt1d(x, wf, bias, out, *, k, u, slope=1.0, algo=ALGO_AUTO, wp=None, stats_part=None, splitk_ws=None):
@@ -439,14 +478,14 @@
     def __init__(self, layers, device):
         n = len(layers)
         self.n = n
-        layers = [tuple(l) + (None,) * (10 - len(l)) for l in layers]
+        layers = [tuple(l) + (None,) * (11 - len(l)) for l in layers]
         rows = [(l[3] if l[7] else l[4]) for l in layers]
         self.scale = torch.empty((sum(rows),), device=device, dtype=torch.float32)
         descs = (_hip.FoldDesc * n)()
         off = 0
-        for d, (v, g, wp, ci, co, k, u, tr, wf, wpd), r in zip(descs, layers, rows):
+        for d, (v, g, wp, ci, co, k, u, tr, wf, wpd, wpw), r in zip(descs, layers, rows):
             d.v = v.data_ptr(); d.g = _hip.ptr(g); d.wp = wp.data_ptr()
-            d.wf = _hip.ptr(wf); d.wpd = _hip.ptr(wpd)
+            d.wf = _hip.ptr(wf); d.wpd = _hip.ptr(wpd); d.wpw = _hip.ptr(wpw)
             d.scale = self.scale.data_ptr() + 4 * off
             d.c_in, d.c_out, d.k, d.u, d.transposed = ci, co, k, u, int(tr)
             off += r
diff --git a/wavthruvec_pytorch_amd/models.py b/wavthruvec_pytorch_amd/models.py
--- a/wavthruvec_pytorch_amd/models.py
+++ b/wavthruvec_pytorch_amd/models.py
@@ -184,6 +184,7 @@
         self.fuse_wide_stage = True
         self.fuse_up = True
         self.fuse_bn_finalize = True
+        self.wino = True
         self.merge_waits = True
         self.cond_stream = None
         self.fuse_post = True
@@ -326,12 +327,14 @@
         for name, m in layers:
             ps = (m.weight_v, m.weight_g) if m.weight_normed else (m.weight,)
             vers.append(tuple((p.data_ptr(), p._version) for p in ps))
-        state = (tuple(vers), self.algo, str(device), need_wf, bf16_only)
+        wino = self.wino and self.precision == 'f32' and self.algo != hipops.ALGO_DIRECT
+        state = (tuple(vers), self.algo, str(device), need_wf, bf16_only, wino)
         force = (self.training and self.always_refold) or need_wf
         if not force and self._fold_key.get('state') == state:
             return self._fold_key['wf'], self._fold_key['wp']
         wf, wp, batch = {}, {}, []
         wpd = {}
+        wpw = {}
         for name, m in layers:
             if bf16_only and name != 'conv_post':
                 wf[name], wp[name] = None, None
@@ -341,6 +344,10 @@
             mfma_ok = (self.algo != hipops.ALGO_DIRECT and name != 'conv_post' and
                        hipops.conv_tile_config(1, m.in_channels, m.out_channels, 64, m.kernel_size,
                                                1 if m.transposed else m.dilation, u) is not None)
+            wpwb = None
+            if (mfma_ok and wino and not m.transposed and hipops.wino_terms(m.kernel_size) and m.in_channels % 32 == 0 and m.in_channels >= 64
+                    and m.out_channels % 64 == 0 and (m.out_channels >= 128 or m.dilation == 1)):
+                wpwb = wpw[name] = self._wbuf('wpw.' + name, (hipops.wino_terms(m.kernel_size) * m.in_channels * m.out_channels,), device=device)
             if mfma_ok and need_wf:
                 n_el = m.kernel_size * m.in_channels * m.out_channels
                 wfb = self._wbuf('wf.' + name, (m.kernel_size, m.in_channels, m.out_channels), device=device)
@@ -348,11 +355,11 @@
                 wdb = None
                 if not m.transposed and m.in_channels == m.out_channels and name.startswith('resblocks.'):
                     wdb = wpd[name] = self._wbuf('wpd.' + name, (n_el,), device=device)
-                batch.append((v, g, wpb, m.in_channels, m.out_channels, m.kernel_size, u, m.transposed, wfb, wdb))
+                batch.append((v, g, wpb, m.in_channels, m.out_channels, m.kernel_size, u, m.transposed, wfb, wdb, wpwb))
                 wf[name], wp[name] = wfb, wpb
             elif mfma_ok:
                 wpb = self._wbuf('wp.' + name, (m.kernel_size * m.in_channels * m.out_channels,), device=device)
-                batch.append((v, g, wpb, m.in_channels, m.out_channels, m.kernel_size, u, m.transposed))
+                batch.append((v, g, wpb, m.in_channels, m.out_channels, m.kernel_size, u, m.transposed, None, None, wpwb))
                 wf[name], wp[name] = None, wpb
             else:
                 wfb = self._wbuf('wf.' + name, (m.kernel_size, m.in_channels, m.out_channels), device=device)
@@ -361,7 +368,7 @@
                 wf[name], wp[name] = wfb, None
         if batch:
             key = tuple((q[0].data_ptr(), 0 if q[1] is None else q[1].data_ptr(), q[2].data_ptr(),
-                         0 if len(q) < 9 or q[8] is None else q[8].data_ptr()) for q in batch)
+                         0 if len(q) < 9 or q[8] is None else q[8].data_ptr(), 0 if len(q) < 11 or q[10] is None else q[10].data_ptr()) for q in batch)
             plan = self._fold_key.get('plan')
             if plan is None or plan.key != key:
                 self._drop_tapes()
@@ -369,7 +376,7 @@
                 plan.key = key
                 self._fold_key['plan'] = plan
             plan.run()
-        self._fold_key.update(state=state, wf=wf, wp=wp, wpd=wpd, vers=tuple(vers), gen=self._fold_key.get('gen', 0) + 1)
+        self._fold_key.update(state=state, wf=wf, wp=wp, wpd=wpd, wpw=wpw, vers=tuple(vers), gen=self._fold_key.get('gen', 0) + 1)
         return wf, wp
 
     def _split_weights(self, device, all_ups=False, ups_stream=None, mark=None, between=None):
@@ -517,7 +524,7 @@
         ptrs = tuple(p.data_ptr() for p in self.parameters()) + tuple(b.data_ptr() for b in self.buffers())
         return (tuple(x.shape), str(x.device), torch.cuda.current_stream(x.device).cuda_stream, self.training, self.precision, self.algo, self.bf16_storage, tuple(self.fuse_stage), tuple(self.fuse_pairs),
                 self.fuse_wide, self.fuse_wide_stage, self.fuse_up, self.fuse_post, self.fuse_bn_finalize, self.cond_stream, self.merge_waits, self.split_min_channels,
-                self.always_refold, ptrs)
+                self.always_refold, self.wino, ptrs)
 
     def _forward_hip(self, x, spk, nz, save):
         from .forward_plan import ForwardPlanner, DirectStreams
```

Measured after the change: 327.1 million samples/s, median of 6. 6.2% higher.
